# yuliangguo/OmniFusion

Measured on AMD Instinct MI355X. Metric: panoramas/sec at 512x1024 ERP, N=18 256^2 patches; equi2pers+pers2equi GB/s vs HBM peak, higher is better.
Workload: dtype f16x3 (fp16 hi/lo pairs, fp32 accumulate: fp32-class); 1 GPU; cfg2/cfg4 shard: 8 panoramas/GPU/step, 512x1024 ERP, fov 80, nrows 4 (18 patches); full single-pass spherical_fusion forward (confidence=True) at patch size 128 — the only size the reference network exists at (SURVEY 0.1); random-init weights (seed 42); inputs resident in HBM; resample pair at 18x256^2 reported in roofline_resample; per_gpu_batch=8, global_batch=8, parallelism=image-sharded x1, execution=3 forwards in flight per GPU on 3 streams (spherical_fusion.pipelined)

## Files before the change

include/omnifusion.h:

```cpp
#ifndef OMNIFUSION_H_
#define OMNIFUSION_H_

#include <stddef.h>
#include <stdint.h>

#ifdef __cplusplus
extern "C" {
#endif

#define OMNI_VERSION 200

enum omni_status {
    OMNI_OK = 0,
    OMNI_ERR_INVALID = 1,
    OMNI_ERR_HIP = 2,
    OMNI_ERR_UNSUPPORTED = 3
};

enum omni_layout { OMNI_LAYOUT_BCHWN = 0, OMNI_LAYOUT_BNCHW = 1, OMNI_LAYOUT_BNHWC = 2,
                   OMNI_LAYOUT_BCHNW = 3  };
enum omni_dtype { OMNI_F32 = 0, OMNI_F16 = 1 };

typedef void* omni_stream_t;
typedef struct omni_geometry omni_geometry_t;

int omni_version(void);
const char* omni_last_error(void);

int omni_set_option(const char* name, int value);
int omni_get_option(const char* name, int* value);

int omni_num_patches(int nrows);

int omni_patch_centers(int nrows, int which, float* center_p_host);

int omni_geometry_create(omni_geometry_t** out, int nrows, float fov_h, float fov_w,
                         int ph, int pw, int H, int W, omni_stream_t stream);
void omni_geometry_destroy(omni_geometry_t* g);
void omni_geometry_cache_clear(void);
int omni_geometry_cache_size(void);

int omni_equi2pers(const void* erp, void* pers, int dtype, int B, int C, int H, int W,
                   int ph, int pw, int nrows, float fov_h, float fov_w, int layout,
                   omni_stream_t stream);

int omni_equi2pers_aux(float* xyz, float* uv, int ph, int pw, int nrows, float fov_h, float fov_w,
                       omni_stream_t stream);

int omni_pers2equi(const void* pers, void* erp, int dtype, int B, int C, int ph, int pw,
                   int H, int W, int nrows, float fov_h, float fov_w, int layout,
                   omni_stream_t stream);

int omni_patches_to_planar(const void* src, void* dst, int dtype, int B, int C, int ph, int pw, int N, omni_stream_t stream);

int omni_pers2equi_conf(const void* pred_w, const void* conf, float* out, int dtype, int B,
                        int ph, int pw, int H, int W, int nrows, float fov_h, float fov_w,
                        int layout, omni_stream_t stream);

int omni_equi2pers_g(const omni_geometry_t* g, const void* erp, void* pers, int dtype, int B, int C,
                     int layout, omni_stream_t stream);
int omni_pers2equi_g(const omni_geometry_t* g, const void* pers, void* erp, int dtype, int B, int C,
                     int layout, omni_stream_t stream);

enum omni_act { OMNI_ACT_NONE = 0, OMNI_ACT_RELU = 1, OMNI_ACT_GELU = 2 };

int omni_equi2pers_bwd(const void* grad_pers, void* grad_erp, int dtype, int B, int C, int H, int W,
                       int ph, int pw, int nrows, float fov_h, float fov_w, int layout, omni_stream_t stream);
int omni_pers2equi_bwd(const void* grad_erp, void* grad_pers, int dtype, int B, int C, int ph, int pw,
                       int H, int W, int nrows, float fov_h, float fov_w, int layout, omni_stream_t stream);
int omni_conv2d_nhwc_f32(const float* src1, const float* src2, const float* wt, const float* bias,
                         const float* res, float* dst, int M, int H, int W, int C1, int C2, int Cout,
                         int KH, int KW, int stride, int pad, int act, omni_stream_t stream);
int omni_conv2d_splitk_plan(long long rows, int Cout, int ksteps);
int omni_conv2d_nhwc_f32_ws(const float* src1, const float* src2, const float* wt, const float* bias,
                            const float* res, float* dst, int M, int H, int W, int C1, int C2, int Cout,
                            int KH, int KW, int stride, int pad, int act, int splitk, float* ws, size_t ws_bytes,
                            omni_stream_t stream);
int omni_conv2d_nhwc_f16x3_ws(const float* src1, const float* src2, const void* wt16, const float* bias,
                              const float* res, float* dst, int M, int H, int W, int C1, int C2, int Cout,
                              int KH, int KW, int stride, int pad, int act, int splitk, float* ws, size_t ws_bytes,
                              omni_stream_t stream);
int omni_conv2d_sh_f16x3_ws(const void* src1, const void* src2, const void* wt16, const float* bias,
                            const void* res, void* dst, int fmt, int M, int H, int W, int C1, int C2, int Cout,
                            int KH, int KW, int stride, int pad, int act, int splitk, float* ws, size_t ws_bytes,
                            omni_stream_t stream);
int omni_gemm_rows_sh_f16x3(const void* x, const void* wt16r, const float* bias, const float* res, void* dst, int fmt,
                            int rows, int K, int N, int act, omni_stream_t stream);
int omni_gemm_rows_pack(const void* wt16, void* wt16r, int N, int K, omni_stream_t stream);
int omni_gemm_rows_ln_sh_f16x3(const float* x, const float* ln_weight, const float* ln_bias, float eps, const void* wt16r, const float* bias,
                               const float* res, void* dst, int fmt, int rows, int N, int act, omni_stream_t stream);
int omni_conv3x3_up2_sh_f16x3(const void* src, const void* wt16, const float* bias, void* dst, int fmt,
                              int M, int Hl, int Wl, int C, int Cout, int act, omni_stream_t stream);
size_t omni_up2_heads_scratch_bytes(int M, int P);
int omni_conv3x3_up2_heads_sh_f16x3(const void* src, const void* wt16, const float* bias, const void* heads_w16f, float bias_pred, float bias_weight,
                                    float* scratch, size_t scratch_bytes, float* out_a, float* out_c, int M, int P, int confidence, omni_stream_t stream);
int omni_conv3x3_up2_heads_sh_f16x1(const void* src, const void* wt16, const float* bias, const void* heads_w16f, float bias_pred, float bias_weight,
                                    float* scratch, size_t scratch_bytes, float* out_a, float* out_c, int M, int P, int confidence, omni_stream_t stream);
int omni_heads_pack_f16x3(const float* w_host, void* dst_host);
int omni_conv2d_sh_f16x3_post_ws(const void* src1, const void* src2, const void* wt16, const float* bias,
                                 const void* res, void* dst, int fmt, int M, int H, int W, int C1, int C2, int Cout,
                                 int KH, int KW, int stride, int pad, int act, int splitk, float* ws, size_t ws_bytes,
                                 const float* post, size_t post_elems, omni_stream_t stream);
int omni_wino_input_sh(const void* src, void* V, int M, int H, int W, int C, omni_stream_t stream);
int omni_conv3x3_wino_sh_f16x3(const void* V, const void* wt16, const float* bias, const void* res, void* dst, int fmt,
                               int M, int H, int W, int C, int Cout, int act, int splitk, float* ws, size_t ws_bytes, omni_stream_t stream);
int omni_sh_from_f32(const float* src, void* dst, size_t n, omni_stream_t stream);
int omni_sh_to_f32(const void* src, float* dst, size_t n, omni_stream_t stream);
int omni_sh_overflow(int* flag, int reset);
int omni_stem_f32(const float* src, const float* wt, const float* bias, float* dst, int M, int P, omni_stream_t stream);
int omni_maxpool3x3s2_f32(const float* src, float* dst, int M, int H, int W, int C, omni_stream_t stream);
int omni_upsample_bilinear_f32(const float* src, float* dst, int M, int H, int W, int C, int Ho, int Wo, omni_stream_t stream);
int omni_add_hw_f32(float* x, const float* y, int M, int HW, int C, omni_stream_t stream);
int omni_add_period_f32(float* x, const float* y, size_t total, size_t period, omni_stream_t stream);
int omni_stem_sh(const float* src, const float* wt, const float* bias, void* dst, int M, int P, omni_stream_t stream);
int omni_stem_sh_f16x3(const float* src, const void* wt16, const float* bias, void* dst, int M, int P, omni_stream_t stream);
int omni_stem_sh_f16x1(const float* src, const void* wt16, const float* bias, void* dst, int M, int P, omni_stream_t stream);
int omni_maxpool3x3s2_sh(const void* src, void* dst, int M, int H, int W, int C, omni_stream_t stream);
int omni_upsample_bilinear_sh(const void* src, void* dst, int M, int H, int W, int C, int Ho, int Wo, omni_stream_t stream);
int omni_up2_tapsum_sh(const float* y, const float* bias, void* dst, int M, int Hl, int Wl, int Cout, int act, omni_stream_t stream);
int omni_add_hw_sh(void* x, const float* y, int M, int HW, int C, omni_stream_t stream);
int omni_add_period_sh(void* x, const float* y, size_t total, size_t period, omni_stream_t stream);
int omni_layernorm512_sh(const float* x, const float* g, const float* b, void* y, int rows, float eps, omni_stream_t stream);
int omni_gemm_rows_slices_sh_f16x3(const void* x, const void* wt16r, float* parts, int rows, int K, int N, int slices, omni_stream_t stream);
int omni_gemm_rows_ln_parts_sh_f16x3(const float* parts, int nparts, const float* pbias, const float* pres, float* xout,
                                     const float* ln_weight, const float* ln_bias, float eps, const void* wt16r, const float* bias,
                                     void* dst, int fmt, int rows, int N, int act, omni_stream_t stream);
int omni_splitk_reduce_ln512(const float* parts, int nparts, const float* bias, const float* res, float* tok, const float* ln_weight, const float* ln_bias,
                             float eps, void* y, int fmt, int rows, omni_stream_t stream);
int omni_gemm_sh_f16x3_ln512_ws(const void* x, const void* wt16, const float* bias, const float* res, float* tok, const float* ln_g, const float* ln_b,
                                float eps, void* y, int fmt, int rows, int K, int splitk, float* ws, size_t ws_bytes, omni_stream_t stream);
int omni_attention_qkv_sh(const float* qkv, void* out, int B, int N, omni_stream_t stream);
int omni_token_pack_f32(const float* d, const float* pos, float* tok, int M, int N, int HW, int C, omni_stream_t stream);
int omni_layernorm512_f32(const float* x, const float* g, const float* b, float* y, int rows, float eps, omni_stream_t stream);
int omni_attention_f32(const float* q, const float* kv, float* out, int B, int N, omni_stream_t stream);
int omni_heads_f32(const float* x, const float* w, float bias_pred, float bias_weight, float* out_a, float* out_c,
                   int M, int P, int confidence, omni_stream_t stream);
int omni_mlp_points_f32(const float* xyz, const float* depth, const float* w1, const float* b1, const float* w2,
                        const float* b2, float* out, int Mo, int N, int HW, omni_stream_t stream);

int omni_masked_median_f32(const float* x, const float* mask, size_t n, unsigned* ws, float* out, omni_stream_t stream);
int omni_depth_metrics_f32(float* pred, const float* gt, const float* mask, const float* scale_num, const float* scale_den,
                           size_t n, double* ws, float* out, omni_stream_t stream);

size_t omni_semantic_workspace_bytes(size_t npix);
int omni_semantic_step_f32(const float* logits, const int64_t* target, int B, int C, size_t HW, int64_t ignore_index, int K,
                           void* workspace, float* loss, int64_t* pred, int64_t* confusion, omni_stream_t stream);
int omni_semantic_grad_f32(const float* logits, const int64_t* target, int B, int C, size_t HW, int64_t ignore_index,
                           const void* workspace, const float* grad_out, float* grad_logits, omni_stream_t stream);
int omni_confusion_matrix_i64(const int64_t* pred, const int64_t* gt, size_t n, int K, int64_t* confusion, int64_t* n_bad,
                              omni_stream_t stream);

int omni_preprocess_rgb_u8(const unsigned char* src_hwc, float* dst_chw, int B, int Hs, int Ws, int H, int W, omni_stream_t stream);
int omni_preprocess_depth_u16(const unsigned short* src, float* depth, unsigned char* mask, int B, int Hs, int Ws, int H, int W,
                              float min_depth, float max_depth, omni_stream_t stream);
int omni_png_info(const void* data, size_t nbytes, int* width, int* height, int* bit_depth, int* color_type);
int omni_png_decode(const void* data, size_t nbytes, void* dst, int H, int W, int kind);
int omni_png_decode_batch(const void* const* datas, const size_t* nbytes, void* const* dsts, int n, int H, int W, int kind, int threads);
int omni_zlib_inflate(const void* src, size_t nbytes, void* dst, size_t cap, size_t* produced, size_t* consumed);
int omni_png_checksums(const void* data, size_t nbytes, unsigned* crc32, unsigned* adler32);
size_t omni_berhu_workspace_bytes(int B);
int omni_berhu_loss_f32(const float* pred, const float* gt, const float* mask, const float* weights, int B, size_t per_item,
                        void* workspace, float* loss, omni_stream_t stream);
int omni_berhu_grad_f32(const float* pred, const float* gt, const float* mask, const float* weights, int B, size_t per_item,
                        const void* workspace, const float* grad_out, float* grad_pred, omni_stream_t stream);
int omni_pointcloud_ply_f32(const float* depth, const float* rgb, unsigned char* records, int B, int H, int W, omni_stream_t stream);

size_t omni_dibr_workspace_bytes(int B, int C, int H, int W);
int omni_splat_render_f32(const float* img, const float* depth, const float* coords, float max_depth,
                          float* recon, unsigned char* mask , int B, int C, int H, int W,
                          void* workspace, omni_stream_t stream);
int omni_dibr_f32(const float* img, const float* depth, const float* uvgrid, const float* sgrid, int grid_batched,
                  float baseline, int mode, float* recon, unsigned char* mask ,
                  int B, int C, int H, int W, void* workspace, omni_stream_t stream);
int omni_splat_render_wt_f32(const float* img, const float* depth, const float* coords, float max_depth,
                             float* recon, unsigned char* mask , float* wt, int B, int C, int H, int W,
                             void* workspace, omni_stream_t stream);
int omni_dibr_wt_f32(const float* img, const float* depth, const float* uvgrid, const float* sgrid, int grid_batched,
                     float baseline, int mode, float* recon, unsigned char* mask , float* wt,
                     int B, int C, int H, int W, void* workspace, omni_stream_t stream);
size_t omni_dibr_bwd_workspace_bytes(int B, int C, int H, int W);
int omni_splat_render_bwd_f32(const float* grad_recon, const float* recon, const float* wt, const float* img, const float* depth,
                              const float* coords, float max_depth, float* grad_img, float* grad_depth, float* grad_coords,
                              int B, int C, int H, int W, void* workspace, omni_stream_t stream);
int omni_dibr_bwd_f32(const float* grad_recon, const float* recon, const float* wt, const float* img, const float* depth,
                      const float* uvgrid, const float* sgrid, int grid_batched, float baseline, int mode,
                      float* grad_img, float* grad_depth, int B, int C, int H, int W, void* workspace, omni_stream_t stream);

int omni_ssim_f32(const float* pred, const float* gt, int B, int C, int H, int W, int window, const float* win, int mode,
                  float* ssim, omni_stream_t stream);
size_t omni_photometric_workspace_bytes(int B, int C, int H, int W);
size_t omni_photometric_grad_scratch_bytes(int B, int C, int H, int W);
int omni_photometric_loss_f32(const float* pred, const float* gt, const float* mask, int mask_c, const float* weights, int weights_c,
                              int B, int C, int H, int W, int window, const float* win, int mode, float alpha,
                              void* workspace, float* loss, omni_stream_t stream);
int omni_photometric_grad_f32(const float* pred, const float* gt, const float* mask, int mask_c, const float* weights, int weights_c,
                              int B, int C, int H, int W, int window, const float* win, int mode, float alpha,
                              const void* workspace, void* scratch, const float* grad_out, float* grad_pred, omni_stream_t stream);

int omni_freeview_rotations(const float* theta_deg, const float* phi_deg, int N, float* rot_fwd_host , float* rot_inv_host );
int omni_freeview_equi2pers_f32(const float* erp, float* pers, const float* rot_fwd_dev, int B, int C, int H, int W,
                                int N, int h, int w, float hfov_deg, float wfov_deg, int layout, omni_stream_t stream);
int omni_freeview_pers2equi_f32(const float* pers, float* erp, unsigned char* mask, const float* rot_inv_dev,
                                int N, int C, int h, int w, int H, int W, float hfov_deg, float wfov_deg, omni_stream_t stream);
int omni_freeview_merge_f32(const float* pers, float* erp, unsigned char* count, const float* rot_inv_dev,
                            int B, int N, int C, int h, int w, int H, int W, float hfov_deg, float wfov_deg, omni_stream_t stream);

size_t omni_freeview_bwd_workspace_bytes(int op, int items, int C, int Ht, int Wt);
int omni_freeview_equi2pers_bwd_f32(const float* grad_pers, float* grad_erp, const float* rot_fwd_dev, int B, int C, int H, int W,
                                    int N, int h, int w, float hfov_deg, float wfov_deg, int layout, void* ws, omni_stream_t stream);
int omni_freeview_pers2equi_bwd_f32(const float* grad_erp, float* grad_pers, const float* rot_inv_dev, int N, int C, int h, int w,
                                    int H, int W, float hfov_deg, float wfov_deg, void* ws, omni_stream_t stream);
int omni_freeview_merge_bwd_f32(const float* grad_erp, float* grad_pers, const float* rot_inv_dev, int B, int N, int C, int h, int w,
                                int H, int W, float hfov_deg, float wfov_deg, void* ws, omni_stream_t stream);

int omni_depth_normals_f32(const float* depth, const float* ray_tables, int B, int H, int W, float* normals, omni_stream_t stream);
int omni_sobel_f32(const float* img, int B, int C, int H, int W, float* grad_y, float* grad_x, omni_stream_t stream);
size_t omni_l1_workspace_bytes(int B);
int omni_l1_loss_f32(const float* pred, const float* gt, const float* mask, int B, int C, size_t hw, int mask_c, void* workspace,
                     float* loss, omni_stream_t stream);
int omni_l1_grad_f32(const float* pred, const float* gt, const float* mask, int B, int C, size_t hw, int mask_c, const void* workspace,
                     const float* grad_out, float* grad_pred, omni_stream_t stream);
size_t omni_geometry_terms_workspace_bytes(int B, int H, int W);
int omni_geometry_terms_f32(const float* pred, const float* gt, const float* mask, const float* ray_tables, int B, int H, int W, int terms,
                            int erode_mask, void* workspace, float* losses, omni_stream_t stream);
int omni_geometry_terms_grad_f32(const float* pred, const float* gt, const float* mask, const float* ray_tables, int B, int H, int W,
                                 int erode_mask, const void* workspace, const float* grad_normal, const float* grad_grad, float* grad_pred,
                                 omni_stream_t stream);

#ifdef __cplusplus
}
#endif
#endif
```

omnifusion_amd/_lib.py:

```python
import ctypes
import os

_HERE = os.path.dirname(os.path.abspath(__file__))
LIB_PATH = os.environ.get("OMNI_LIB_VARIANT") or os.path.join(_HERE, "csrc", "libomnifusion_hip.so")
LIB_PATH_DEBUG = os.path.join(_HERE, "csrc", "libomnifusion_hip_dbg.so")

OMNI_OK, OMNI_ERR_INVALID, OMNI_ERR_HIP, OMNI_ERR_UNSUPPORTED = 0, 1, 2, 3
LAYOUT_BCHWN, LAYOUT_BNCHW, LAYOUT_BNHWC, LAYOUT_BCHNW = 0, 1, 2, 3
F32, F16 = 0, 1

_lib = None


class OmniLibraryMissing(ImportError):
    pass


EXPORTS = [
    "omni_version", "omni_last_error", "omni_set_option", "omni_get_option", "omni_num_patches", "omni_patch_centers",
    "omni_geometry_create", "omni_geometry_destroy", "omni_geometry_cache_clear", "omni_geometry_cache_size",
    "omni_equi2pers", "omni_equi2pers_aux", "omni_pers2equi", "omni_pers2equi_conf", "omni_patches_to_planar",
    "omni_equi2pers_g", "omni_pers2equi_g", "omni_equi2pers_bwd", "omni_pers2equi_bwd",
    "omni_conv2d_nhwc_f32", "omni_stem_f32", "omni_maxpool3x3s2_f32", "omni_upsample_bilinear_f32",
    "omni_add_hw_f32", "omni_add_period_f32", "omni_token_pack_f32", "omni_layernorm512_f32",
    "omni_attention_f32", "omni_heads_f32", "omni_mlp_points_f32",
    "omni_conv2d_nhwc_f16x3_ws", "omni_conv2d_sh_f16x3_ws", "omni_conv2d_sh_f16x3_post_ws", "omni_gemm_rows_sh_f16x3", "omni_gemm_rows_ln_sh_f16x3", "omni_gemm_rows_pack", "omni_conv3x3_up2_sh_f16x3", "omni_conv3x3_up2_heads_sh_f16x3", "omni_conv3x3_up2_heads_sh_f16x1", "omni_up2_heads_scratch_bytes", "omni_heads_pack_f16x3", "omni_sh_from_f32", "omni_sh_to_f32", "omni_sh_overflow",
    "omni_stem_sh", "omni_stem_sh_f16x3", "omni_stem_sh_f16x1", "omni_maxpool3x3s2_sh", "omni_upsample_bilinear_sh", "omni_up2_tapsum_sh", "omni_add_hw_sh", "omni_add_period_sh", "omni_layernorm512_sh", "omni_gemm_sh_f16x3_ln512_ws", "omni_gemm_rows_slices_sh_f16x3", "omni_gemm_rows_ln_parts_sh_f16x3", "omni_splitk_reduce_ln512", "omni_wino_input_sh", "omni_conv3x3_wino_sh_f16x3", "omni_attention_qkv_sh",
    "omni_conv2d_splitk_plan", "omni_conv2d_nhwc_f32_ws",
    "omni_masked_median_f32", "omni_depth_metrics_f32",
    "omni_png_info", "omni_png_decode", "omni_png_decode_batch", "omni_zlib_inflate", "omni_png_checksums",
    "omni_preprocess_rgb_u8", "omni_preprocess_depth_u16", "omni_berhu_workspace_bytes", "omni_berhu_loss_f32", "omni_berhu_grad_f32",
    "omni_pointcloud_ply_f32",
    "omni_dibr_workspace_bytes", "omni_splat_render_f32", "omni_dibr_f32",
    "omni_splat_render_wt_f32", "omni_dibr_wt_f32", "omni_dibr_bwd_workspace_bytes", "omni_splat_render_bwd_f32", "omni_dibr_bwd_f32",
    "omni_ssim_f32", "omni_photometric_workspace_bytes", "omni_photometric_grad_scratch_bytes", "omni_photometric_loss_f32",
    "omni_photometric_grad_f32",
    "omni_freeview_rotations", "omni_freeview_equi2pers_f32", "omni_freeview_pers2equi_f32", "omni_freeview_merge_f32",
    "omni_freeview_bwd_workspace_bytes", "omni_freeview_equi2pers_bwd_f32", "omni_freeview_pers2equi_bwd_f32", "omni_freeview_merge_bwd_f32",
    "omni_semantic_workspace_bytes", "omni_semantic_step_f32", "omni_semantic_grad_f32", "omni_confusion_matrix_i64",
    "omni_depth_normals_f32", "omni_sobel_f32", "omni_l1_workspace_bytes", "omni_l1_loss_f32", "omni_l1_grad_f32",
    "omni_geometry_terms_workspace_bytes", "omni_geometry_terms_f32", "omni_geometry_terms_grad_f32",
]


def load():
    global _lib
    if _lib is not None:
        return _lib
    if not os.path.exists(LIB_PATH):
        raise OmniLibraryMissing(
            f"{LIB_PATH} not found: build it with `python -m omnifusion_amd.build` "
            "(hipcc --offload-arch=gfx950).  There is no fallback path.")
    import torch
    lib = ctypes.CDLL(LIB_PATH)
    lib.omni_last_error.restype = ctypes.c_char_p
    lib.omni_version.restype = ctypes.c_int
    lib.omni_up2_heads_scratch_bytes.restype = ctypes.c_size_t
    lib.omni_dibr_workspace_bytes.restype = ctypes.c_size_t
    lib.omni_splat_render_f32.argtypes = [ctypes.c_void_p] * 3 + [ctypes.c_float] + [ctypes.c_void_p] * 2 + [ctypes.c_int] * 4 + [ctypes.c_void_p] * 2
    lib.omni_dibr_f32.argtypes = [ctypes.c_void_p] * 4 + [ctypes.c_int, ctypes.c_float, ctypes.c_int] + [ctypes.c_void_p] * 2 + \
        [ctypes.c_int] * 4 + [ctypes.c_void_p] * 2
    vp, ci, cf = ctypes.c_void_p, ctypes.c_int, ctypes.c_float
    lib.omni_splat_render_wt_f32.argtypes = [vp] * 3 + [cf] + [vp] * 3 + [ci] * 4 + [vp] * 2
    lib.omni_dibr_wt_f32.argtypes = [vp] * 4 + [ci, cf, ci] + [vp] * 3 + [ci] * 4 + [vp] * 2
    lib.omni_dibr_bwd_workspace_bytes.restype = ctypes.c_size_t
    lib.omni_splat_render_bwd_f32.argtypes = [vp] * 6 + [cf] + [vp] * 3 + [ci] * 4 + [vp] * 2
    lib.omni_dibr_bwd_f32.argtypes = [vp] * 7 + [ci, cf, ci] + [vp] * 2 + [ci] * 4 + [vp] * 2
    lib.omni_ssim_f32.argtypes = [vp] * 2 + [ci] * 5 + [vp, ci, vp, vp]
    lib.omni_photometric_workspace_bytes.restype = ctypes.c_size_t
    lib.omni_photometric_grad_scratch_bytes.restype = ctypes.c_size_t
    lib.omni_photometric_loss_f32.argtypes = [vp, vp, vp, ci, vp, ci] + [ci] * 5 + [vp, ci, cf] + [vp] * 3
    lib.omni_photometric_grad_f32.argtypes = [vp, vp, vp, ci, vp, ci] + [ci] * 5 + [vp, ci, cf] + [vp] * 5
    lib.omni_freeview_rotations.argtypes = [vp, vp, ci, vp, vp]
    lib.omni_freeview_equi2pers_f32.argtypes = [vp] * 3 + [ci] * 7 + [cf, cf, ci, vp]
    lib.omni_freeview_pers2equi_f32.argtypes = [vp] * 4 + [ci] * 6 + [cf, cf, vp]
    lib.omni_freeview_merge_f32.argtypes = [vp] * 4 + [ci] * 7 + [cf, cf, vp]
    lib.omni_freeview_bwd_workspace_bytes.restype = ctypes.c_size_t
    lib.omni_freeview_bwd_workspace_bytes.argtypes = [ci] * 5
    lib.omni_freeview_equi2pers_bwd_f32.argtypes = [vp] * 3 + [ci] * 7 + [cf, cf, ci, vp, vp]
    lib.omni_freeview_pers2equi_bwd_f32.argtypes = [vp] * 3 + [ci] * 6 + [cf, cf, vp, vp]
    lib.omni_freeview_merge_bwd_f32.argtypes = [vp] * 3 + [ci] * 7 + [cf, cf, vp, vp]
    sz, i64 = ctypes.c_size_t, ctypes.c_int64
    lib.omni_semantic_workspace_bytes.restype = sz
    lib.omni_semantic_workspace_bytes.argtypes = [sz]
    lib.omni_semantic_step_f32.argtypes = [vp, vp, ci, ci, sz, i64, ci] + [vp] * 5
    lib.omni_semantic_grad_f32.argtypes = [vp, vp, ci, ci, sz, i64] + [vp] * 4
    lib.omni_confusion_matrix_i64.argtypes = [vp, vp, sz, ci] + [vp] * 3
    lib.omni_depth_normals_f32.argtypes = [vp, vp, ci, ci, ci, vp, vp]
    lib.omni_sobel_f32.argtypes = [vp] + [ci] * 4 + [vp] * 3
    lib.omni_l1_workspace_bytes.restype = sz
    lib.omni_l1_workspace_bytes.argtypes = [ci]
    lib.omni_l1_loss_f32.argtypes = [vp] * 3 + [ci, ci, sz, ci] + [vp] * 3
    lib.omni_l1_grad_f32.argtypes = [vp] * 3 + [ci, ci, sz, ci] + [vp] * 4
    lib.omni_geometry_terms_workspace_bytes.restype = sz
    lib.omni_geometry_terms_workspace_bytes.argtypes = [ci] * 3
    lib.omni_geometry_terms_f32.argtypes = [vp] * 4 + [ci] * 5 + [vp] * 3
    lib.omni_geometry_terms_grad_f32.argtypes = [vp] * 4 + [ci] * 4 + [vp] * 5
    for name in EXPORTS:
        getattr(lib, name)
    _lib = lib
    return lib


def load_debug():
    import torch
    if not os.path.exists(LIB_PATH_DEBUG):
        raise OmniLibraryMissing(f"{LIB_PATH_DEBUG} not found: python -m omnifusion_amd.build --debug")
    lib = ctypes.CDLL(LIB_PATH_DEBUG)
    lib.omni_last_error.restype = ctypes.c_char_p
    return lib


def set_option(name, value):
    check(load().omni_set_option(name.encode(), int(value)), "set_option")


def get_option(name):
    v = ctypes.c_int(0)
    check(load().omni_get_option(name.encode(), ctypes.byref(v)), "get_option")
    return v.value


CALL_LOG = None


def check(status, what=""):
    if CALL_LOG is not None:
        CALL_LOG.append(what)
    if status == OMNI_OK:
        return
    msg = load().omni_last_error().decode(errors="replace")
    if status == OMNI_ERR_INVALID:
        raise ValueError(f"{what}: {msg}")
    if status == OMNI_ERR_UNSUPPORTED:
        raise NotImplementedError(f"{what}: {msg}")
    raise RuntimeError(f"{what}: {msg}")


def ptr(t):
    return ctypes.c_void_p(t.data_ptr())


def stream_of(t):
    import torch
    return ctypes.c_void_p(torch.cuda.current_stream(t.device).cuda_stream)


def dtype_code(t):
    import torch
    if t.dtype == torch.float32:
        return F32
    if t.dtype == torch.float16:
        return F16
    raise ValueError(f"unsupported dtype {t.dtype}: the HIP path stores float32 or float16")
```

omnifusion_amd/csrc/omni_conv_sh.hip:

```cpp
#include "omni_conv_sh_common.h"

namespace {

__constant__ float wino_coef[16][4] = {
    {1, 0, 0, 0}, {1, 1, 0, 0}, {1, -1, 0, 0}, {0, -1, 0, 0},
    {1, 0, 1, 0}, {1, 1, 1, 1}, {1, -1, 1, -1}, {0, -1, 0, -1},
    {1, 0, -1, 0}, {1, 1, -1, -1}, {1, -1, -1, 1}, {0, -1, 0, 1},
    {0, 0, -1, 0}, {0, 0, -1, -1}, {0, 0, -1, 1}, {0, 0, 0, 1}};
template <int BM, int BN, int WM, int WN, int NST = 3, int NL = 0, bool PP = false, bool WINO = false, bool X1 = false>
__global__ __launch_bounds__(64 * (WM * WN + NL)) void conv_sh_kernel(ShConvArgs a)
{
    static_assert(!(WINO && X1), "Winograd: f16x3 only");
    static_assert(!PP || (NL > 0 && WM * WN == 8 && NST >= 3), "ping-pong: eight matrix waves (two per SIMD) + loader waves, three stages");
    static_assert(!WINO || (PP && BM / WM == 32 && BN / WN == 32), "Winograd: the ping-pong kernel with 32 x 32 wave tiles");
    constexpr int NW = WM * WN, LW = NL > 0 ? NL : NW, RPP = 8 * LW;
    constexpr int TM = BM / WM / 32, TN = BN / WN / 32;
    constexpr int APASS = BM / RPP, BPASS = BN / RPP, LPS = APASS + BPASS;
    static_assert(APASS >= 1 && BPASS >= 1, "a tile side must cover at least one DMA pass");
    constexpr int A_BYTES = BM * 128, STAGE = (BM + BN) * 128;
    __shared__ __attribute__((aligned(1024))) unsigned char lds[NST * STAGE];
    __shared__ long long cst[OMNI_ABL(32768) ? 256 : 1];
    const bool stamped = OMNI_ABL(32768) && blockIdx.x == 0 && blockIdx.y == 0 && a.ws != nullptr && a.splitk <= 1;
    auto cstamp = [&](int k) { if (OMNI_ABL(32768) && stamped && (threadIdx.x & 63) == 0 && k < 256) cst[k] = clock64(); };
    auto cdump = [&]() { if (OMNI_ABL(32768) && stamped && threadIdx.x == 0) for (int i = 0; i < 256; ++i) reinterpret_cast<long long*>(a.ws)[i] = cst[i]; };
    if (threadIdx.x == 0) cstamp(0);

    const int t = threadIdx.x, lane = t & 63;
    const int wave = __builtin_amdgcn_readfirstlane(t >> 6);
    const int wm = wave / WN, wn = wave % WN;
    const bool loader = NL > 0 && wave >= NW;
    const int iw = NL > 0 ? wave - NW : wave;
    const int ntn = a.Cout / BN;
    const int ntm = (a.rows + BM - 1) / BM;
    const unsigned lb = a.noxcd ? blockIdx.x : omni_xcd_remap(blockIdx.x, gridDim.x);
    const int tile_m = a.wt_major ? (int)(lb % (unsigned)ntm) : (int)(lb / (unsigned)ntn), tile_n = a.wt_major ? (int)(lb / (unsigned)ntm) : (int)(lb % (unsigned)ntn);
    const int row0 = tile_m * BM, col0 = tile_n * BN;
    const int G1 = a.C1 >> 5, G2 = a.C2 >> 5, G = G1 + G2;
    const int ksteps = a.KH * a.KW * G;

    const int gs = (lane & 15) ^ ((4 * iw + (lane >> 4)) & 15);
    const int rl = 8 * iw + 2 * (lane >> 4) + (gs >> 3), pc16 = (gs & 7) * 16;
    int pix[APASS];
    unsigned vmask[APASS];
#pragma unroll
    for (int i = 0; i < APASS; ++i) {
        const int r = row0 + rl + RPP * i;
        vmask[i] = 0; pix[i] = 0;
        if constexpr (WINO) {
            if ((NL == 0 || loader) && r < a.rows) { pix[i] = r; vmask[i] = 0xffffu; }
        } else
        if ((NL == 0 || loader) && r < a.rows) {
            const int hw = a.Ho * a.Wo;
            const int m = r / hw, rem = r - m * hw;
            const int oy = (rem / a.Wo) * a.stride - a.pad, ox = (rem % a.Wo) * a.stride - a.pad;
            pix[i] = (m * a.H + oy) * a.W + ox;
            unsigned vm = 0;
#pragma unroll
            for (int ky = 0; ky < 3; ++ky)
#pragma unroll
                for (int kx = 0; kx < 3; ++kx)
                    if (ky < a.KH && kx < a.KW && (unsigned)(oy + ky) < (unsigned)a.H && (unsigned)(ox + kx) < (unsigned)a.W)
                        vm |= 1u << (ky * a.KW + kx);
            vmask[i] = vm;
        }
    }
    const rsrc_t rs1 = make_rsrc(a.src1, (size_t)a.M * a.H * a.W * a.C1 * 4);
    const rsrc_t rs2 = make_rsrc(a.src2 ? a.src2 : a.src1, a.src2 ? (size_t)a.M * a.H * a.W * a.C2 * 4 : 0);
    const rsrc_t rsw = make_rsrc(a.wt, (size_t)a.Cout * ksteps * 128);
    int wbase[BPASS];
#pragma unroll
    for (int i = 0; i < BPASS; ++i) wbase[i] = (col0 + rl + RPP * i) * ksteps * 128 + pc16;

    int f_tap = 0, f_src = 0, f_gl = 0, f_ky = 0, f_kx = 0, f_gn = G1;
    int voff[APASS];
    auto refresh = [&]() {
        const int cs4 = (f_src ? a.C2 : a.C1) * 4;
        const int toff = (f_ky * a.W + f_kx) * cs4 + pc16;
#pragma unroll
        for (int i = 0; i < APASS; ++i)
            voff[i] = ((vmask[i] >> f_tap) & 1u) ? pix[i] * cs4 + toff : (int)0x80000000;
    };
    auto seek = [&](int ks) {
        f_tap = ks / G; const int g = ks - f_tap * G;
        f_src = g >= G1; f_gl = f_src ? g - G1 : g; f_gn = f_src ? G2 : G1;
        f_ky = f_tap / a.KW; f_kx = f_tap - f_ky * a.KW;
        refresh();
    };
    auto issue_a = [&](auto slot_c) {
        constexpr int SLOT = decltype(slot_c)::value;
        unsigned char* sb = lds + SLOT * STAGE + iw * 1024;
        const int so = f_gl * 128;
        if (OMNI_ABL(128)) {}
        else if (f_src) {
#pragma unroll
            for (int i = 0; i < APASS; ++i) dma16(rs2, sb + i * (1024 * LW), voff[i], so);
        } else {
#pragma unroll
            for (int i = 0; i < APASS; ++i) dma16(rs1, sb + i * (1024 * LW), voff[i], so);
        }
    };
    auto issue_b = [&](int ks, auto slot_c) {
        constexpr int SLOT = decltype(slot_c)::value;
        unsigned char* sb = lds + SLOT * STAGE + iw * 1024;
        if (!OMNI_ABL(128)) {
#pragma unroll
            for (int i = 0; i < BPASS; ++i) dma16(rsw, sb + A_BYTES + i * (1024 * LW), wbase[i], ks * 128);
        }
        if (++f_gl == f_gn) {
            f_gl = 0;
            if (f_src == 0 && G2 > 0) { f_src = 1; f_gn = G2; }
            else { f_src = 0; f_gn = G1; ++f_tap; if (++f_kx == a.KW) { f_kx = 0; ++f_ky; } }
            refresh();
        }
    };
    auto issue = [&](int ks, auto slot_c) { issue_a(slot_c); issue_b(ks, slot_c); };

    f16v acc[TM][TN], acc1[TM][TN];
#pragma unroll
    for (int i = 0; i < TM; ++i)
#pragma unroll
        for (int j = 0; j < TN; ++j) { acc[i][j] = (f16v)(0.0f); acc1[i][j] = (f16v)(0.0f); }

    int foa[4], fob[4];
    {
        const int r = lane & 31, v = r >> 1, h = lane >> 5;
#pragma unroll
        for (int k = 0; k < 4; ++k) {
            const int f = v * 256 + ((((r & 1) * 8 + 2 * k + h) ^ v) * 16);
            foa[k] = f + wm * (BM / WM) * 128;
            fob[k] = f + A_BYTES + wn * (BN / WN) * 128;
        }
    }

    int ks_begin = 0, ks_end = ksteps;
    if (a.splitk > 1) {
        const int per = (ksteps + a.splitk - 1) / a.splitk;
        ks_begin = (int)blockIdx.y * per; ks_end = min(ksteps, ks_begin + per);
    }
    if (NL == 0 || loader) {
        seek(ks_begin);
        [&]<int... S>(std::integer_sequence<int, S...>) {
            ((ks_begin + S < ks_end ? issue(ks_begin + S, std::integral_constant<int, S>()) : (void)0), ...);
        }(std::make_integer_sequence<int, NST - 1>());
    }
    auto pbarrier = [&]() {
        __builtin_amdgcn_sched_barrier(0);
        __builtin_amdgcn_s_barrier();
        asm volatile("" ::: "memory");
        __builtin_amdgcn_sched_barrier(0);
    };
    if (loader) {
        if constexpr (PP) {
            auto lstep = [&](int ks, auto slot_c) {
                constexpr int SLOT = decltype(slot_c)::value;
                const int sk_ = 128 + 4 * (ks - ks_begin);
                if (wave == NW && ks - ks_begin < 28) cstamp(sk_);
                if (ks + NST - 2 < ks_end) wait_vm<(NST - 2) * LPS>();
                else                       wait_vm<0>();
                if (wave == NW && ks - ks_begin < 28) cstamp(sk_ + 1);
                pbarrier();
                if (wave == NW && ks - ks_begin < 28) cstamp(sk_ + 2);
                if (ks + NST - 1 < ks_end) issue_a(std::integral_constant<int, (SLOT + NST - 1) % NST>());
                if (wave == NW && ks - ks_begin < 28) cstamp(sk_ + 3);
                pbarrier();
                if (ks + NST - 1 < ks_end) issue_b(ks + NST - 1, std::integral_constant<int, (SLOT + NST - 1) % NST>());
            };
            int ks = ks_begin;
            for (; ks + NST - 1 < ks_end; ks += NST) {
                [&]<int... S>(std::integer_sequence<int, S...>) { (lstep(ks + S, std::integral_constant<int, S>()), ...); }
                (std::make_integer_sequence<int, NST>());
            }
            [&]<int... S>(std::integer_sequence<int, S...>) {
                ((ks + S < ks_end ? lstep(ks + S, std::integral_constant<int, S>()) : (void)0), ...);
            }(std::make_integer_sequence<int, NST - 1>());
            pbarrier();
            if (!WINO && a.splitk <= 1 && a.dst_sh && !a.res_f32 && !a.post && a.epi_lds) __syncthreads();
            return;
        }
        auto lstep = [&](int ks, auto slot_c) {
            constexpr int SLOT = decltype(slot_c)::value;
            const int sk_ = 128 + 4 * (ks - ks_begin);
            if (wave == NW && ks - ks_begin < 28) cstamp(sk_);
            if (ks + NST - 2 < ks_end) wait_vm<(NST - 2) * LPS>();
            else                       wait_vm<0>();
            if (wave == NW && ks - ks_begin < 28) cstamp(sk_ + 1);
            __builtin_amdgcn_s_barrier();
            asm volatile("" ::: "memory");
            if (wave == NW && ks - ks_begin < 28) cstamp(sk_ + 2);
            if (ks + NST - 1 < ks_end) issue(ks + NST - 1, std::integral_constant<int, (SLOT + NST - 1) % NST>());
            if (wave == NW && ks - ks_begin < 28) cstamp(sk_ + 3);
        };
        int ks = ks_begin;
        for (; ks + NST - 1 < ks_end; ks += NST) {
            [&]<int... S>(std::integer_sequence<int, S...>) { (lstep(ks + S, std::integral_constant<int, S>()), ...); }
            (std::make_integer_sequence<int, NST>());
        }
        [&]<int... S>(std::integer_sequence<int, S...>) {
            ((ks + S < ks_end ? lstep(ks + S, std::integral_constant<int, S>()) : (void)0), ...);
        }(std::make_integer_sequence<int, NST - 1>());
        if (a.splitk <= 1 && a.dst_sh && !a.res_f32 && !a.post && a.epi_lds) __syncthreads();
        return;
    }

    if constexpr (PP) {
        const bool grp_b = wave >= NW / 2;
        h8v ah[2][TM], al[2][TM], bh[2][TN], bl[2][TN];
        auto reads = [&](auto slot_c) {
            constexpr int SLOT = decltype(slot_c)::value;
            const unsigned char* sl = lds + SLOT * STAGE;
#pragma unroll
            for (int kc = 0; kc < 2; ++kc) {
#pragma unroll
                for (int i = 0; i < TM; ++i) {
                    ah[kc][i] = *reinterpret_cast<const h8v*>(sl + i * 4096 + foa[kc]);
                    if constexpr (!X1) al[kc][i] = *reinterpret_cast<const h8v*>(sl + i * 4096 + foa[2 + kc]);
                }
#pragma unroll
                for (int j = 0; j < TN; ++j) {
                    bh[kc][j] = *reinterpret_cast<const h8v*>(sl + j * 4096 + fob[kc]);
                    if constexpr (!X1) bl[kc][j] = *reinterpret_cast<const h8v*>(sl + j * 4096 + fob[2 + kc]);
                }
            }
            wait_lds_reads();
        };
        auto mfmas = [&]() {
            if constexpr (OMNI_PP_PRIO) __builtin_amdgcn_s_setprio(1);
#pragma unroll
            for (int kc = 0; kc < 2; ++kc)
#pragma unroll
                for (int i = 0; i < TM; ++i)
#pragma unroll
                    for (int j = 0; j < TN; ++j) {
                        acc[i][j] = __builtin_amdgcn_mfma_f32_32x32x16_f16(bh[kc][j], ah[kc][i], acc[i][j], 0, 0, 0);
                        if constexpr (!X1) {
                            acc1[i][j] = __builtin_amdgcn_mfma_f32_32x32x16_f16(bl[kc][j], ah[kc][i], acc1[i][j], 0, 0, 0);
                            acc1[i][j] = __builtin_amdgcn_mfma_f32_32x32x16_f16(bh[kc][j], al[kc][i], acc1[i][j], 0, 0, 0);
                        }
                    }
            if constexpr (OMNI_PP_PRIO) __builtin_amdgcn_s_setprio(0);
        };
        f16v Y[WINO ? 4 : 1];
        int wino_g = 0, wino_p = ks_begin / (G > 0 ? G : 1);
        if constexpr (WINO) {
#pragma unroll
            for (int o = 0; o < 4; ++o) Y[o] = (f16v)(0.0f);
        }
        auto wino_fold = [&]() {
            if constexpr (WINO) {
                if (++wino_g < G) return;
                wino_g = 0;
                f16v m;
#pragma unroll
                for (int e = 0; e < 16; ++e) m[e] = fmaf(acc1[0][0][e], 4.8828125e-4f, acc[0][0][e]);
#pragma unroll
                for (int o = 0; o < 4; ++o) {
                    const float c = wino_coef[wino_p][o];
                    if (c != 0.0f) {
#pragma unroll
                        for (int e = 0; e < 16; ++e) Y[o][e] = fmaf(c, m[e], Y[o][e]);
                    }
                }
                acc[0][0] = (f16v)(0.0f); acc1[0][0] = (f16v)(0.0f);
                ++wino_p;
            }
        };
        pbarrier();
        if (!grp_b) {
            auto stepa = [&](int ks, auto slot_c) {
                if (wave == 0 && ks - ks_begin < 28) cstamp(8 + 4 * (ks - ks_begin));
                reads(slot_c);
                if (wave == 0 && ks - ks_begin < 28) cstamp(11 + 4 * (ks - ks_begin));
                pbarrier();
                if (wave == 0 && ks - ks_begin < 28) cstamp(9 + 4 * (ks - ks_begin));
                mfmas();
                wino_fold();
                if (wave == 0 && ks - ks_begin < 28) cstamp(10 + 4 * (ks - ks_begin));
                pbarrier();
            };
            int ks = ks_begin;
            for (; ks + NST - 1 < ks_end; ks += NST) {
                [&]<int... S>(std::integer_sequence<int, S...>) { (stepa(ks + S, std::integral_constant<int, S>()), ...); }
                (std::make_integer_sequence<int, NST>());
            }
            [&]<int... S>(std::integer_sequence<int, S...>) {
                ((ks + S < ks_end ? stepa(ks + S, std::integral_constant<int, S>()) : (void)0), ...);
            }(std::make_integer_sequence<int, NST - 1>());
        } else {
            auto stepb = [&](int ks, auto slot_c) {
                pbarrier();
                reads(slot_c);
                pbarrier();
                mfmas();
                wino_fold();
            };
            int ks = ks_begin;
            for (; ks + NST - 1 < ks_end; ks += NST) {
                [&]<int... S>(std::integer_sequence<int, S...>) { (stepb(ks + S, std::integral_constant<int, S>()), ...); }
                (std::make_integer_sequence<int, NST>());
            }
            [&]<int... S>(std::integer_sequence<int, S...>) {
                ((ks + S < ks_end ? stepb(ks + S, std::integral_constant<int, S>()) : (void)0), ...);
            }(std::make_integer_sequence<int, NST - 1>());
        }
        if constexpr (WINO) {
            const int tl = row0 + wm * (BM / WM) + (lane & 31);
            if (tl >= a.rows) return;
            const int per_img = a.wino_th * a.wino_tw, m = tl / per_img, rem = tl - m * per_img, ty = rem / a.wino_tw, tx = rem - ty * a.wino_tw;
            const int cj[1] = {col0 + wn * (BN / WN)};
#pragma unroll
            for (int o = 0; o < 4; ++o) {
                const size_t r = ((size_t)m * a.Ho + 2 * ty + (o >> 1)) * a.Wo + 2 * tx + (o & 1);
                if (a.splitk > 1) {
#pragma unroll
                    for (int q = 0; q < 4; ++q) {
                        f4v v; v.x = Y[o][4 * q]; v.y = Y[o][4 * q + 1]; v.z = Y[o][4 * q + 2]; v.w = Y[o][4 * q + 3];
                        *reinterpret_cast<f4v*>(a.ws + ((size_t)blockIdx.y * a.wino_pix + r) * a.Cout + cj[0] + 8 * q + 4 * (lane >> 5)) = v;
                    }
                } else {
                    const f16v ea[1] = {Y[o]}, eb[1] = {(f16v)(0.0f)};
                    epilogue_row<1, 2>(ea, eb, a, r, cj, lane, a.dst_sh != 0);
                }
            }
            return;
        }
    }
    auto step = [&](int ks, auto slot_c) {
        constexpr int SLOT = decltype(slot_c)::value;
        if (NL == 0) {
            if (ks + NST - 2 < ks_end) wait_vm<(NST - 2) * LPS>();
            else                       wait_vm<0>();
        }
        if (wave == 0 && ks - ks_begin < 28) cstamp(8 + 4 * (ks - ks_begin));
        wait_lds_reads();
        if (!OMNI_ABL(256)) __builtin_amdgcn_s_barrier();
        asm volatile("" ::: "memory");
        if (wave == 0 && ks - ks_begin < 28) cstamp(9 + 4 * (ks - ks_begin));
        const unsigned char* sl = lds + SLOT * STAGE;
        h8v ah[2][TM], al[2][TM], bh[2][TN], bl[2][TN];
        if (OMNI_ABL(512)) {
#pragma unroll
            for (int kc = 0; kc < 2; ++kc) {
#pragma unroll
                for (int i = 0; i < TM; ++i) { ah[kc][i] = (h8v)((_Float16)1.0f); al[kc][i] = ah[kc][i]; }
#pragma unroll
                for (int j = 0; j < TN; ++j) { bh[kc][j] = (h8v)((_Float16)1.0f); bl[kc][j] = bh[kc][j]; }
            }
        } else
#pragma unroll
        for (int kc = 0; kc < 2; ++kc) {
#pragma unroll
            for (int i = 0; i < TM; ++i) {
                ah[kc][i] = *reinterpret_cast<const h8v*>(sl + i * 4096 + foa[kc]);
                if constexpr (!X1) al[kc][i] = *reinterpret_cast<const h8v*>(sl + i * 4096 + foa[2 + kc]);
            }
#pragma unroll
            for (int j = 0; j < TN; ++j) {
                bh[kc][j] = *reinterpret_cast<const h8v*>(sl + j * 4096 + fob[kc]);
                if constexpr (!X1) bl[kc][j] = *reinterpret_cast<const h8v*>(sl + j * 4096 + fob[2 + kc]);
            }
        }
#pragma unroll
        for (int kc = 0; kc < 2; ++kc) {
            __builtin_amdgcn_sched_barrier(0);
#pragma unroll
            for (int i = 0; i < TM; ++i)
#pragma unroll
                for (int j = 0; j < TN; ++j) {
                    if (!OMNI_ABL(64) && !OMNI_DBG(a, 64)) acc[i][j] = __builtin_amdgcn_mfma_f32_32x32x16_f16(bh[kc][j], ah[kc][i], acc[i][j], 0, 0, 0);
                    else { acc[i][j][0] += (float)bh[kc][j][0] * (float)ah[kc][i][0]; }
                    if constexpr (!X1) {
                        if (!OMNI_ABL(16) && !OMNI_DBG(a, 16)) acc1[i][j] = __builtin_amdgcn_mfma_f32_32x32x16_f16(bl[kc][j], ah[kc][i], acc1[i][j], 0, 0, 0);
                        if (!OMNI_ABL(32) && !OMNI_DBG(a, 32)) acc1[i][j] = __builtin_amdgcn_mfma_f32_32x32x16_f16(bh[kc][j], al[kc][i], acc1[i][j], 0, 0, 0);
                    }
                }
            if (kc == 0) {
                __builtin_amdgcn_sched_barrier(0);
                if (NL == 0 && ks + NST - 1 < ks_end) issue(ks + NST - 1, std::integral_constant<int, (SLOT + NST - 1) % NST>());
            }
        }
    };
    if constexpr (!PP) {
        int ks = ks_begin;
        for (; ks + NST - 1 < ks_end; ks += NST) {
            [&]<int... S>(std::integer_sequence<int, S...>) { (step(ks + S, std::integral_constant<int, S>()), ...); }
            (std::make_integer_sequence<int, NST>());
        }
        [&]<int... S>(std::integer_sequence<int, S...>) {
            ((ks + S < ks_end ? step(ks + S, std::integral_constant<int, S>()) : (void)0), ...);
        }(std::make_integer_sequence<int, NST - 1>());
    }

    if (wave == 0) cstamp(1);
    if (OMNI_ABL(4) || OMNI_DBG(a, 4)) return;
    if (a.splitk <= 1 && a.dst_sh && !a.res_f32 && !a.post && a.epi_lds) {
        static_assert(NW * 32 * (32 * TN + 4) * 4 <= NST * STAGE, "the transposition tiles must fit the K loop's buffers");
        wait_lds_reads();
        __syncthreads();
        float* tile = reinterpret_cast<float*>(lds) + wave * (32 * (32 * TN + 4));
        int c0[TN];
#pragma unroll
        for (int j = 0; j < TN; ++j) c0[j] = col0 + wn * (BN / WN) + j * 32;
#pragma unroll
        for (int i = 0; i < TM; ++i) {
            const int r0 = row0 + wm * (BM / WM) + i * 32;
            if (r0 < a.rows) epilogue_tile_lds<TN, false, X1>(acc[i], acc1[i], a, (size_t)r0, min(32, a.rows - r0), c0, lane, tile);
            if (i + 1 < TM) asm volatile("s_waitcnt lgkmcnt(0)" ::: "memory");
        }
        if (OMNI_ABL(32768)) { if (wave == 0) cstamp(2); __syncthreads(); cdump(); }
        return;
    }
#pragma unroll
    for (int i = 0; i < TM; ++i) {
        const int r = row0 + wm * (BM / WM) + i * 32 + (lane & 31);
        if (r >= a.rows) continue;
        if (a.splitk > 1) {
#pragma unroll
            for (int j = 0; j < TN; ++j)
#pragma unroll
                for (int q = 0; q < 4; ++q) {
                    const int c = col0 + wn * (BN / WN) + j * 32 + 8 * q + 4 * (lane >> 5);
                    f4v v;
#pragma unroll
                    for (int e = 0; e < 4; ++e) v[e] = acc_join<X1>(acc1[i][j][4 * q + e], acc[i][j][4 * q + e]);
                    *reinterpret_cast<f4v*>(a.ws + ((size_t)blockIdx.y * a.rows + r) * a.Cout + c) = v;
                }
        } else {
            if constexpr (NL > 0 && TN > 1) {
#pragma unroll
                for (int j = 0; j < TN; ++j) {
                    const f16v ea[1] = {acc[i][j]}, eb[1] = {acc1[i][j]};
                    const int cj[1] = {col0 + wn * (BN / WN) + j * 32};
                    epilogue_row<1, 2, X1>(ea, eb, a, (size_t)r, cj, lane, a.dst_sh != 0);
                }
            } else {
                int c0[TN];
#pragma unroll
                for (int j = 0; j < TN; ++j) c0[j] = col0 + wn * (BN / WN) + j * 32;
                epilogue_row<TN, 4, X1>(acc[i], acc1[i], a, (size_t)r, c0, lane, a.dst_sh != 0);
            }
        }
    }
}

__global__ __launch_bounds__(256) void sh_splitk_reduce_kernel(const float* __restrict__ ws, const float* __restrict__ bias,
                                                               const void* __restrict__ res, void* __restrict__ dst,
                                                               size_t n4, int Cout, int splitk, size_t slab, int act, int dst_sh, int res_f32)
{
    const size_t i = (size_t)blockIdx.x * 256 + threadIdx.x;
    if (i >= n4) return;
    const size_t o = i * 4;
    f4v v = *reinterpret_cast<const f4v*>(ws + o);
    for (int s = 1; s < splitk; ++s) v += *reinterpret_cast<const f4v*>(ws + (size_t)s * slab + o);
    splitk_finish(v, o, bias, res, dst, Cout, act, dst_sh, res_f32);
}

template <bool SH>
__global__ __launch_bounds__(256) void sh_splitk_reduce_ln512_kernel(const float* __restrict__ ws, const float* __restrict__ bias, const float* __restrict__ res,
                                                                     float* __restrict__ tok, const float* __restrict__ g, const float* __restrict__ b,
                                                                     void* __restrict__ y, int rows, int splitk, size_t slab, float eps)
{
    const int row = blockIdx.x * 4 + (threadIdx.x >> 6), lane = threadIdx.x & 63;
    if (row >= rows) return;
    const size_t o = (size_t)row * 512;
    f4v v0 = *reinterpret_cast<const f4v*>(ws + o + lane * 4), v1 = *reinterpret_cast<const f4v*>(ws + o + 256 + lane * 4);
    for (int s = 1; s < splitk; ++s) {
        v0 += *reinterpret_cast<const f4v*>(ws + (size_t)s * slab + o + lane * 4);
        v1 += *reinterpret_cast<const f4v*>(ws + (size_t)s * slab + o + 256 + lane * 4);
    }
    if (bias) { v0 += *reinterpret_cast<const f4v*>(bias + lane * 4); v1 += *reinterpret_cast<const f4v*>(bias + 256 + lane * 4); }
    if (res) { v0 += *reinterpret_cast<const f4v*>(res + o + lane * 4); v1 += *reinterpret_cast<const f4v*>(res + o + 256 + lane * 4); }
    *reinterpret_cast<f4v*>(tok + o + lane * 4) = v0; *reinterpret_cast<f4v*>(tok + o + 256 + lane * 4) = v1;
    float sum = (v0.x + v0.y) + (v0.z + v0.w) + (v1.x + v1.y) + (v1.z + v1.w);
#pragma unroll
    for (int d = 32; d > 0; d >>= 1) sum += __shfl_xor(sum, d);
    const float mean = sum * (1.0f / 512.0f);
    v0 -= mean; v1 -= mean;
    float q = (v0.x * v0.x + v0.y * v0.y) + (v0.z * v0.z + v0.w * v0.w) + (v1.x * v1.x + v1.y * v1.y) + (v1.z * v1.z + v1.w * v1.w);
#pragma unroll
    for (int d = 32; d > 0; d >>= 1) q += __shfl_xor(q, d);
    const float rstd = 1.0f / sqrtf(q * (1.0f / 512.0f) + eps);
    const f4v g0 = *reinterpret_cast<const f4v*>(g + lane * 4), g1 = *reinterpret_cast<const f4v*>(g + 256 + lane * 4);
    const f4v b0 = *reinterpret_cast<const f4v*>(b + lane * 4), b1 = *reinterpret_cast<const f4v*>(b + 256 + lane * 4);
    act_store4<SH>(y, o + lane * 4, v0 * rstd * g0 + b0);
    act_store4<SH>(y, o + 256 + lane * 4, v1 * rstd * g1 + b1);
}

__global__ __launch_bounds__(256) void sh_from_f32_kernel(const float* __restrict__ src, void* __restrict__ dst, size_t n4)
{
    const size_t i = (size_t)blockIdx.x * 256 + threadIdx.x;
    if (i >= n4) return;
    h4v hi, lo; sh_split4(*reinterpret_cast<const f4v*>(src + i * 4), hi, lo);
    unsigned char* dp = (unsigned char*)dst + sh_off(i * 4);
    *reinterpret_cast<h4v*>(dp) = hi; *reinterpret_cast<h4v*>(dp + 64) = lo;
}
__global__ __launch_bounds__(256) void sh_to_f32_kernel(const void* __restrict__ src, float* __restrict__ dst, size_t n4)
{
    const size_t i = (size_t)blockIdx.x * 256 + threadIdx.x;
    if (i >= n4) return;
    const unsigned char* sp = (const unsigned char*)src + sh_off(i * 4);
    *reinterpret_cast<f4v*>(dst + i * 4) = sh_join4(*reinterpret_cast<const h4v*>(sp), *reinterpret_cast<const h4v*>(sp + 64));
}

template <bool X1, int BM, int BN, int WM, int WN, int NST = 3, int NL = 0>
void launch_sh(ShConvArgs a, hipStream_t s)
{
    const int tiles = ((a.rows + BM - 1) / BM) * (a.Cout / BN);
    if constexpr (NL > 0 && WM * WN == 8) {
        if (omni_options().conv_pingpong) {
            hipLaunchKernelGGL((conv_sh_kernel<BM, BN, WM, WN, NST, NL, true, false, X1>), dim3(tiles, a.splitk > 1 ? a.splitk : 1), dim3(64 * (WM * WN + NL)), 0, s, a);
            return;
        }
    }
    hipLaunchKernelGGL((conv_sh_kernel<BM, BN, WM, WN, NST, NL, false, false, X1>), dim3(tiles, a.splitk > 1 ? a.splitk : 1), dim3(64 * (WM * WN + NL)), 0, s, a);
}

}

static int conv2d_sh_impl(const void* src1, const void* src2, const void* wt16, const float* bias,
                          const void* res, void* dst, int fmt, int M, int H, int W, int C1, int C2, int Cout,
                          int KH, int KW, int stride, int pad, int act, int splitk, float* ws, size_t ws_bytes,
                          const float* post, size_t post_elems, omni_stream_t stream, bool reduce = true);
extern "C" int omni_conv2d_sh_f16x3_ws(const void* src1, const void* src2, const void* wt16, const float* bias,
                                       const void* res, void* dst, int fmt, int M, int H, int W, int C1, int C2, int Cout,
                                       int KH, int KW, int stride, int pad, int act, int splitk, float* ws, size_t ws_bytes,
                                       omni_stream_t stream)
{
    return conv2d_sh_impl(src1, src2, wt16, bias, res, dst, fmt, M, H, W, C1, C2, Cout, KH, KW, stride, pad, act, splitk, ws, ws_bytes,
                          nullptr, 0, stream);
}
extern "C" int omni_conv2d_sh_f16x3_post_ws(const void* src1, const void* src2, const void* wt16, const float* bias,
                                            const void* res, void* dst, int fmt, int M, int H, int W, int C1, int C2, int Cout,
                                            int KH, int KW, int stride, int pad, int act, int splitk, float* ws, size_t ws_bytes,
                                            const float* post, size_t post_elems, omni_stream_t stream)
{
    return conv2d_sh_impl(src1, src2, wt16, bias, res, dst, fmt, M, H, W, C1, C2, Cout, KH, KW, stride, pad, act, splitk, ws, ws_bytes,
                          post, post_elems, stream);
}
extern "C" int omni_gemm_sh_f16x3_ln512_ws(const void* x, const void* wt16, const float* bias, const float* res, float* tok, const float* ln_g, const float* ln_b,
                                           float eps, void* y, int fmt, int rows, int K, int splitk, float* ws, size_t ws_bytes, omni_stream_t stream)
{
    if (!x || !wt16 || !tok || !ln_g || !ln_b || !y) OMNI_FAIL(OMNI_ERR_INVALID, "omni_gemm_sh_f16x3_ln512: null pointer");
    if (rows <= 0 || K <= 0 || K % 32) OMNI_FAIL(OMNI_ERR_INVALID, "omni_gemm_sh_f16x3_ln512: bad shape");
    if (fmt & 8) OMNI_FAIL(OMNI_ERR_UNSUPPORTED, "omni_gemm_sh_f16x3_ln512: no f16x1 form (fmt bit 3)");
    const int S = std::min(splitk, K / 32);
    if (S < 2) OMNI_FAIL(OMNI_ERR_INVALID, "omni_gemm_sh_f16x3_ln512: needs a split-K plan (splitk >= 2); an unsplit GEMM writes its result in its own epilogue");
    const int rc = conv2d_sh_impl(x, nullptr, wt16, bias, res, tok, 2, rows, 1, 1, K, 0, 512, 1, 1, 1, 0, OMNI_ACT_NONE, S, ws, ws_bytes, nullptr, 0, stream, false);
    if (rc != OMNI_OK) return rc;
    hipStream_t s = (hipStream_t)stream;
    if (fmt & 1) hipLaunchKernelGGL(sh_splitk_reduce_ln512_kernel<true>, dim3((rows + 3) / 4), dim3(256), 0, s, (const float*)ws, bias, res, tok, ln_g, ln_b, y, rows, S, (size_t)rows * 512, eps);
    else         hipLaunchKernelGGL(sh_splitk_reduce_ln512_kernel<false>, dim3((rows + 3) / 4), dim3(256), 0, s, (const float*)ws, bias, res, tok, ln_g, ln_b, y, rows, S, (size_t)rows * 512, eps);
    OMNI_HIP(hipGetLastError());
    return OMNI_OK;
}

template <bool X1>
static void conv_sh_select(const ShConvArgs& a, int fmt, hipStream_t s)
{
    const int KH = a.KH, KW = a.KW, stride = a.stride, pad = a.pad, H = a.H, W = a.W, M = a.M, Cout = a.Cout;
    const int ksteps = KH * KW * ((a.C1 + a.C2) / 32);
    const long long rows = a.rows;
    if (a.splitk <= 1 && KH == 3 && KW == 3 && stride == 1 && pad == 1 && H == W && (W == 16 || (W == 8 && omni_options().conv_img >= 2)) && rows % 128 == 0 &&
        Cout % 64 == 0 && !(fmt & 4) && omni_options().conv_img > 0 && !omni_options().conv_nohalo) {
        const int grid = (int)(rows / 128) * (Cout / 64);
        if (omni_options().conv_halo_bn == 32) {
            if (W == 16) omni_halo_launch(&a, 32, 4, false, 16, X1, 2 * grid, s);
            else         omni_halo_launch(&a, 32, 4, false, 8, X1, 2 * grid, s);
        }
        else if (W == 16) omni_halo_launch(&a, 64, 4, false, 16, X1, grid, s);
        else         omni_halo_launch(&a, 64, 4, false, 8, X1, grid, s);
        return;
    }
    if (a.splitk <= 1 && KH == 3 && KW == 3 && stride == 1 && pad == 1 && W % HT_W == 0 && H % 4 == 0 && !omni_options().conv_nohalo) {
        const int th = (H % 8 == 0 && omni_options().conv_halo_th == 8) ? 8 : 4;
        const int grid = M * (H / th) * (W / HT_W);
        if (th == 8) {
            if (Cout % 64 == 0 && omni_options().conv_halo_bn != 32) omni_halo_launch(&a, 64, 8, false, 0, X1, grid * (Cout / 64), s);
            else                omni_halo_launch(&a, 32, 8, false, 0, X1, grid * (Cout / 32), s);
        } else {
            const bool bn32 = omni_options().conv_halo_bn == 32 || ((fmt & 4) && omni_options().conv_halo_bn_lat == 32);
            if (Cout % 64 == 0 && !bn32) omni_halo_launch(&a, 64, 4, false, 0, X1, grid * (Cout / 64), s);
            else                omni_halo_launch(&a, 32, 4, false, 0, X1, grid * (Cout / 32), s);
        }
        return;
    }
    int tile = omni_options().conv_sh_tile;
    if (tile < 0) tile = 8;
    if (Cout % 64 != 0) launch_sh<X1, 128, 32, 4, 1>(a, s);
    else if (tile == 2 && Cout % 128 == 0) launch_sh<X1, 128, 128, 2, 2>(a, s);
    else if (tile == 1) launch_sh<X1, 128, 64, 2, 2>(a, s);
    else if (tile == 3) launch_sh<X1, 128, 64, 4, 2>(a, s);
    else if (tile == 4 && Cout % 128 == 0) launch_sh<X1, 128, 128, 4, 2>(a, s);
    else if (tile == 8 && Cout % 128 == 0 && ((rows + 255) / 256) * (long long)(Cout / 128) * a.splitk >= std::max(1, omni_options().conv_big_blocks)) launch_sh<X1, 256, 128, 4, 2>(a, s);
    else if (tile == 8 && Cout % 128 == 0 && ((rows + 127) / 128) * (long long)(Cout / 128) * a.splitk >= 128) launch_sh<X1, 128, 128, 4, 2, 3, 4>(a, s);
    else if (tile == 8 && ((rows + 127) / 128) * (long long)(Cout / 64) * a.splitk >= 128) launch_sh<X1, 128, 64, 4, 2, 3, 4>(a, s);
    else if (tile == 9 && Cout % 128 == 0 && ((rows + 255) / 256) * (long long)(Cout / 128) * a.splitk >= 128) launch_sh<X1, 256, 128, 4, 2>(a, s);
    else if (tile == 9 && Cout % 128 == 0 && ((rows + 127) / 128) * (long long)(Cout / 128) * a.splitk >= 128) launch_sh<X1, 128, 128, 4, 2>(a, s);
    else if (tile == 9 && ((rows + 127) / 128) * (long long)(Cout / 64) * a.splitk >= 128) launch_sh<X1, 128, 64, 4, 2>(a, s);
    else if (tile >= 5 && tile <= 7 && Cout % 128 == 0 && ((rows + 127) / 128) * (long long)(Cout / 128) * a.splitk >= (32ll << (tile - 4))) launch_sh<X1, 128, 128, 4, 2>(a, s);
    else if (tile >= 5 && tile <= 7 && ((rows + 127) / 128) * (long long)(Cout / 64) * a.splitk >= (32ll << (tile - 4))) launch_sh<X1, 128, 64, 4, 2>(a, s);
    else if (((rows + 63) / 64) * (long long)(Cout / 64) * a.splitk <= 256 && ksteps >= 8 && !omni_options().conv_nodeep) {
        if (omni_options().conv_deep_loaders) launch_sh<X1, 64, 64, 2, 2, 6, 4>(a, s);
        else launch_sh<X1, 64, 64, 2, 2, 6>(a, s);
    }
    else launch_sh<X1, 64, 64, 2, 2>(a, s);
}

static int conv2d_sh_impl(const void* src1, const void* src2, const void* wt16, const float* bias,
                          const void* res, void* dst, int fmt, int M, int H, int W, int C1, int C2, int Cout,
                          int KH, int KW, int stride, int pad, int act, int splitk, float* ws, size_t ws_bytes,
                          const float* post, size_t post_elems, omni_stream_t stream, bool reduce)
{
    const int dst_sh = fmt & 1;
    if (!src1 || !wt16 || !dst) OMNI_FAIL(OMNI_ERR_INVALID, "omni_conv2d_sh: null pointer");
    if (C1 <= 0 || C1 % 32 || C2 < 0 || C2 % 32 || Cout <= 0 || Cout % 32 || (C2 > 0 && !src2))
        OMNI_FAIL(OMNI_ERR_INVALID, "omni_conv2d_sh: channels must be multiples of 32");
    if (M <= 0 || H <= 0 || W <= 0 || KH <= 0 || KW <= 0 || KH > 3 || KW > 3 || stride <= 0 || pad < 0)
        OMNI_FAIL(OMNI_ERR_INVALID, "omni_conv2d_sh: bad shape (kernels up to 3x3)");
    ShConvArgs a;
    a.src1 = src1; a.src2 = src2; a.wt = wt16; a.bias = bias; a.res = res; a.dst = dst; a.dst_sh = dst_sh; a.res_f32 = (fmt >> 1) & 1;
    a.dbg = 0; a.noxcd = omni_options().conv_noxcd; a.wt_major = 0; a.epi_lds = omni_options().conv_epi_lds && !(fmt & 4);
#ifdef OMNI_DEBUG_BUILD
    a.dbg = omni_debug_bits("OMNI_CONV_DBG");
#endif
    a.M = M; a.H = H; a.W = W; a.C1 = C1; a.C2 = C2; a.Cout = Cout;
    a.KH = KH; a.KW = KW; a.stride = stride; a.pad = pad; a.act = act;
    a.Ho = (H + 2 * pad - KH) / stride + 1; a.Wo = (W + 2 * pad - KW) / stride + 1;
    const long long rows = (long long)M * a.Ho * a.Wo;
    if (rows <= 0 || rows >= (1ll << 31) || (long long)M * H * W >= (1ll << 31))
        OMNI_FAIL(OMNI_ERR_UNSUPPORTED, "omni_conv2d_sh: too many pixels for 32-bit row indices");
    a.rows = (int)rows;
    const int ksteps = KH * KW * ((C1 + C2) / 32);
    if ((long long)M * H * W * (C1 > C2 ? C1 : C2) * 4 >= (1ll << 31) || (long long)Cout * ksteps * 128 >= (1ll << 31))
        OMNI_FAIL(OMNI_ERR_UNSUPPORTED, "omni_conv2d_sh: an operand of 2 GiB or more (32-bit buffer offsets)");
    int S = splitk;
    if (S > ksteps) S = ksteps;
    if (S > 1 && (!ws || ws_bytes < (size_t)S * rows * Cout * sizeof(float)))
        OMNI_FAIL(OMNI_ERR_INVALID, "omni_conv2d_sh: split-K workspace too small");
    a.splitk = S > 1 ? S : 1; a.ws = ws;
    a.wt_major = omni_options().conv_wt_major == 2 || (omni_options().conv_wt_major == 1 &&
                 (long long)Cout * ksteps * 128 > (long long)M * H * W * (C1 + C2) * 4) ? 1 : 0;
    a.post = post; a.post_rows = 1; a.wino_th = a.wino_tw = a.wino_pix = 0;
    if (post) {
        if (Cout <= 0 || post_elems == 0 || post_elems % (size_t)Cout || post_elems / (size_t)Cout > 0x7fffffffull)
            OMNI_FAIL(OMNI_ERR_INVALID, "omni_conv2d_sh: the post-activation addend must hold whole rows of Cout channels");
        if (a.splitk > 1) OMNI_FAIL(OMNI_ERR_UNSUPPORTED, "omni_conv2d_sh: no post-activation addend with split-K");
        a.post_rows = (unsigned)(post_elems / (size_t)Cout);
    }
    hipStream_t s = (hipStream_t)stream;
    if (fmt & 8) conv_sh_select<true>(a, fmt, s);
    else         conv_sh_select<false>(a, fmt, s);
    OMNI_HIP(hipGetLastError());
    if (a.splitk > 1 && reduce) {
        const size_t n4 = (size_t)rows * Cout / 4;
        hipLaunchKernelGGL(sh_splitk_reduce_kernel, dim3((unsigned)((n4 + 255) / 256)), dim3(256), 0, s, (const float*)ws, bias, res, dst,
                           n4, Cout, a.splitk, (size_t)rows * Cout, act, a.dst_sh, a.res_f32);
        OMNI_HIP(hipGetLastError());
    }
    return OMNI_OK;
}

extern "C" int omni_splitk_reduce_ln512(const float* parts, int nparts, const float* bias, const float* res, float* tok, const float* lg, const float* lb,
                                        float eps, void* y, int fmt, int rows, omni_stream_t stream)
{
    if (!parts || nparts < 1 || !tok || !lg || !lb || !y || rows <= 0) OMNI_FAIL(OMNI_ERR_INVALID, "omni_splitk_reduce_ln512: null pointer or empty input");
    hipStream_t s = (hipStream_t)stream;
    if (fmt & 1) hipLaunchKernelGGL(sh_splitk_reduce_ln512_kernel<true>, dim3((rows + 3) / 4), dim3(256), 0, s, parts, bias, res, tok, lg, lb, y, rows, nparts, (size_t)rows * 512, eps);
    else         hipLaunchKernelGGL(sh_splitk_reduce_ln512_kernel<false>, dim3((rows + 3) / 4), dim3(256), 0, s, parts, bias, res, tok, lg, lb, y, rows, nparts, (size_t)rows * 512, eps);
    OMNI_HIP(hipGetLastError());
    return OMNI_OK;
}

OMNI_SH_OVERFLOW_ACCESSOR(omni_sh_overflow_conv)

extern "C" int omni_sh_overflow(int* flag, int reset)
{
    if (!flag) OMNI_FAIL(OMNI_ERR_INVALID, "omni_sh_overflow: null output");
    OMNI_HIP(hipDeviceSynchronize());
    unsigned v = 0;
    if (omni_sh_overflow_conv(&v, reset) != 0 || omni_sh_overflow_halo(&v, reset) != 0 || omni_sh_overflow_up2(&v, reset) != 0 ||
        omni_sh_overflow_rows(&v, reset) != 0 || omni_sh_overflow_net(&v, reset) != 0)
        OMNI_FAIL(OMNI_ERR_HIP, "omni_sh_overflow: could not read the device flag");
    *flag = v ? 1 : 0;
    return OMNI_OK;
}

extern "C" int omni_sh_from_f32(const float* src, void* dst, size_t n, omni_stream_t stream)
{
    if (!src || !dst || n % 32) OMNI_FAIL(OMNI_ERR_INVALID, "omni_sh_from_f32: null pointer or n % 32 != 0");
    if (n == 0) return OMNI_OK;
    hipLaunchKernelGGL(sh_from_f32_kernel, dim3((unsigned)((n / 4 + 255) / 256)), dim3(256), 0, (hipStream_t)stream, src, dst, n / 4);
    OMNI_HIP(hipGetLastError());
    return OMNI_OK;
}
extern "C" int omni_sh_to_f32(const void* src, float* dst, size_t n, omni_stream_t stream)
{
    if (!src || !dst || n % 32) OMNI_FAIL(OMNI_ERR_INVALID, "omni_sh_to_f32: null pointer or n % 32 != 0");
    if (n == 0) return OMNI_OK;
    hipLaunchKernelGGL(sh_to_f32_kernel, dim3((unsigned)((n / 4 + 255) / 256)), dim3(256), 0, (hipStream_t)stream, src, dst, n / 4);
    OMNI_HIP(hipGetLastError());
    return OMNI_OK;
}

namespace {

__global__ __launch_bounds__(256) void wino_input_sh_kernel(const void* __restrict__ src, void* __restrict__ V, int M, int H, int W, int C, size_t nt)
{
    const size_t i = (size_t)blockIdx.x * 256 + threadIdx.x;
    const int cq = C >> 2;
    if (i >= nt * cq) return;
    const size_t tl = i / cq;
    const int c = (int)(i - tl * cq) * 4;
    const int tw = W >> 1, th = H >> 1;
    const int m = (int)(tl / (size_t)(th * tw)), rem = (int)(tl - (size_t)m * th * tw), ty = rem / tw, tx = rem - ty * tw;
    f4v d[4][4];
#pragma unroll
    for (int a_ = 0; a_ < 4; ++a_)
#pragma unroll
        for (int b_ = 0; b_ < 4; ++b_) {
            const int y = 2 * ty - 1 + a_, x = 2 * tx - 1 + b_;
            d[a_][b_] = ((unsigned)y < (unsigned)H && (unsigned)x < (unsigned)W) ? act_load4<true>(src, (((size_t)m * H + y) * W + x) * C + c) : (f4v)(0.0f);
        }
    f4v u[4][4];
#pragma unroll
    for (int b_ = 0; b_ < 4; ++b_) { u[0][b_] = d[0][b_] - d[2][b_]; u[1][b_] = d[1][b_] + d[2][b_]; u[2][b_] = d[2][b_] - d[1][b_]; u[3][b_] = d[1][b_] - d[3][b_]; }
#pragma unroll
    for (int xi = 0; xi < 4; ++xi) {
        const f4v v0 = u[xi][0] - u[xi][2], v1 = u[xi][1] + u[xi][2], v2 = u[xi][2] - u[xi][1], v3 = u[xi][1] - u[xi][3];
        act_store4<true>(V, ((size_t)(4 * xi + 0) * nt + tl) * C + c, v0);
        act_store4<true>(V, ((size_t)(4 * xi + 1) * nt + tl) * C + c, v1);
        act_store4<true>(V, ((size_t)(4 * xi + 2) * nt + tl) * C + c, v2);
        act_store4<true>(V, ((size_t)(4 * xi + 3) * nt + tl) * C + c, v3);
    }
}

}

extern "C" int omni_wino_input_sh(const void* src, void* V, int M, int H, int W, int C, omni_stream_t stream)
{
    if (!src || !V) OMNI_FAIL(OMNI_ERR_INVALID, "omni_wino_input_sh: null pointer");
    if (M <= 0 || H <= 0 || W <= 0 || (H & 1) || (W & 1) || C <= 0 || C % 32) OMNI_FAIL(OMNI_ERR_INVALID, "omni_wino_input_sh: even image sides, channels a multiple of 32");
    const size_t nt = (size_t)M * (H / 2) * (W / 2), n = nt * (C / 4);
    if (16 * nt * C * 4 >= (1ull << 31)) OMNI_FAIL(OMNI_ERR_UNSUPPORTED, "omni_wino_input_sh: the transformed tensor must stay under 2 GiB (32-bit buffer offsets)");
    hipLaunchKernelGGL(wino_input_sh_kernel, dim3((unsigned)((n + 255) / 256)), dim3(256), 0, (hipStream_t)stream, src, V, M, H, W, C, nt);
    OMNI_HIP(hipGetLastError());
    return OMNI_OK;
}

extern "C" int omni_conv3x3_wino_sh_f16x3(const void* V, const void* wt16, const float* bias, const void* res, void* dst, int fmt,
                                          int M, int H, int W, int C, int Cout, int act, int splitk, float* ws, size_t ws_bytes, omni_stream_t stream)
{
    if (!V || !wt16 || !dst) OMNI_FAIL(OMNI_ERR_INVALID, "omni_conv3x3_wino_sh: null pointer");
    if (M <= 0 || H <= 0 || W <= 0 || (H & 1) || (W & 1) || C <= 0 || C % 32 || Cout <= 0 || Cout % 64) OMNI_FAIL(OMNI_ERR_INVALID, "omni_conv3x3_wino_sh: even image sides, C % 32 == 0, Cout % 64 == 0");
    if (splitk != 1 && splitk != 2 && splitk != 4) OMNI_FAIL(OMNI_ERR_INVALID, "omni_conv3x3_wino_sh: splitk must be 1, 2 or 4 (it divides the sixteen positions)");
    if (fmt & 8) OMNI_FAIL(OMNI_ERR_UNSUPPORTED, "omni_conv3x3_wino_sh: no f16x1 form (fmt bit 3)");
    const long long nt = (long long)M * (H / 2) * (W / 2), pix = (long long)M * H * W;
    if (16 * nt * C * 4 >= (1ll << 31) || (long long)Cout * 16 * C * 4 >= (1ll << 31) || pix >= (1ll << 31)) OMNI_FAIL(OMNI_ERR_UNSUPPORTED, "omni_conv3x3_wino_sh: an operand of 2 GiB or more");
    if (splitk > 1 && (!ws || ws_bytes < (size_t)splitk * pix * Cout * sizeof(float))) OMNI_FAIL(OMNI_ERR_INVALID, "omni_conv3x3_wino_sh: split workspace too small");
    ShConvArgs a;
    a.src1 = V; a.src2 = nullptr; a.wt = wt16; a.bias = bias; a.res = res; a.dst = dst; a.dst_sh = fmt & 1; a.res_f32 = (fmt >> 1) & 1;
    a.dbg = 0; a.noxcd = omni_options().conv_noxcd; a.wt_major = 0; a.epi_lds = 0;
    a.M = 1; a.H = 16; a.W = (int)nt; a.C1 = C; a.C2 = 0; a.Cout = Cout; a.KH = 16; a.KW = 1; a.stride = 1; a.pad = 0; a.act = act;
    a.Ho = H; a.Wo = W; a.rows = (int)nt; a.splitk = splitk; a.ws = ws; a.post = nullptr; a.post_rows = 1;
    a.wino_th = H / 2; a.wino_tw = W / 2; a.wino_pix = (int)pix;
    hipStream_t s = (hipStream_t)stream;
    const int tiles = (int)((nt + 127) / 128) * (Cout / 64);
    hipLaunchKernelGGL((conv_sh_kernel<128, 64, 4, 2, 3, 4, true, true>), dim3(tiles, splitk), dim3(64 * 12), 0, s, a);
    OMNI_HIP(hipGetLastError());
    if (splitk > 1) {
        const size_t n4 = (size_t)pix * Cout / 4;
        hipLaunchKernelGGL(sh_splitk_reduce_kernel, dim3((unsigned)((n4 + 255) / 256)), dim3(256), 0, s, (const float*)ws, bias, res, dst,
                           n4, Cout, splitk, (size_t)pix * Cout, act, a.dst_sh, a.res_f32);
        OMNI_HIP(hipGetLastError());
    }
    return OMNI_OK;
}
```

omnifusion_amd/model/_engine.py:

```python
import ctypes
import os

import torch

from .. import _lib
from ..equi_pers.equi2pers_v3 import equi2pers_patches, equi2pers_aux, pair, _NPATCH
from ..equi_pers.pers2equi_v3 import pers2equi, pers2equi_conf

ACT_NONE, ACT_RELU, ACT_GELU = 0, 1, 2
_LAYERS = [("layer1", 3, 1), ("layer2", 4, 2), ("layer3", 6, 2), ("layer4", 3, 2)]
_BN_EPS = 1e-5
PRECISIONS = ("f16x3", "f16x1", "fp32")


def _p(t):
    return ctypes.c_void_p(t.data_ptr()) if t is not None else None


def split_weights_f16x3(w):
    w = w.to(torch.float32)
    wmax = float(w.abs().max()) if w.numel() else 0.0
    if not wmax < 65504.0:
        raise ValueError(f"folded weight magnitude {wmax:g} is outside the fp16 range of the f16x3 operand format: "
                         "run this checkpoint with OMNI_NET_PRECISION=fp32")
    hi = w.half()
    hi = torch.where(w.abs() < 6.103515625e-05, torch.zeros_like(hi), hi)
    lo = ((w - hi.float()) * 2048.0).half()
    co, k = w.shape
    return torch.stack([hi.reshape(co, k // 32, 32), lo.reshape(co, k // 32, 32)], 2).contiguous()


def strip_module_prefix(sd):
    return {(k[7:] if k.startswith("module.") else k): v for k, v in sd.items()}


class Engine:
    def __init__(self, nrows, npatches, patch_size, fov, iterative, precision=None):
        self.nrows, self.npatches, self.iterative = nrows, npatches, iterative
        self.patch_size = pair(patch_size)
        self.fov = pair(fov)
        if self.patch_size[0] != self.patch_size[1]:
            raise ValueError("square patches only")
        self.w = None
        self.device = None
        self.precision = precision if precision is not None else os.environ.get("OMNI_NET_PRECISION", "f16x3")

    @property
    def sh(self):
        return self.precision in ("f16x3", "f16x1")

    @property
    def terms(self):
        return {"f16x3": 3, "f16x1": 1}.get(self.precision, 0)

    @property
    def _x1(self):
        return 8 if self.terms == 1 else 0

    def lane(self):
        e = Engine(self.nrows, self.npatches, self.patch_size, self.fov, self.iterative, precision=self.precision)
        e.w, e.device, e.head_bias = self.w, self.device, getattr(self, "head_bias", None)
        return e

    @staticmethod
    def _fold(sd, conv, bn):
        w = sd[conv + ".weight"].double()
        if w.dim() == 5:
            w = w[..., 0]
        g = sd[bn + ".weight"].double() / torch.sqrt(sd[bn + ".running_var"].double() + _BN_EPS)
        b = sd[bn + ".bias"].double() - sd[bn + ".running_mean"].double() * g
        return w * g[:, None, None, None], b

    @staticmethod
    def _gemm_layout(w):
        return w.permute(0, 2, 3, 1).reshape(w.shape[0], -1)

    def pack(self, state_dict, device):
        sd = {k: v.detach().cpu() for k, v in strip_module_prefix(state_dict).items()}
        dev = torch.device(device)
        f = lambda t: t.to(torch.float32).contiguous().to(dev)
        W = {}
        w, b = self._fold(sd, "conv1", "bn1")
        W["stem.w"] = f(w.permute(2, 3, 1, 0).reshape(147, 64)); W["stem.b"] = f(b)
        wk = torch.zeros((64, 3, 7, 8), dtype=torch.float64); wk[..., :7] = w
        W["stem.w16"] = split_weights_f16x3(torch.cat([wk.reshape(64, 168), torch.zeros((64, 24), dtype=torch.float64)], 1)).to(dev)

        def convbn(key, conv, bn):
            w, b = self._fold(sd, conv, bn)
            wg = self._gemm_layout(w).to(torch.float32)
            W[key + ".w"] = f(wg); W[key + ".b"] = f(b)
            W[key + ".w16"] = split_weights_f16x3(wg).to(dev)
        for lname, nblk, _ in _LAYERS:
            for i in range(nblk):
                p = f"{lname}.{i}"
                convbn(p + ".c1", p + ".conv1", p + ".bn1")
                convbn(p + ".c2", p + ".conv2", p + ".bn2")
                if (p + ".downsample.0.weight") in sd:
                    convbn(p + ".ds", p + ".downsample.0", p + ".downsample.1")
        for name in ("de_conv0_0", "de_conv0_1", "de_conv1_0", "de_conv1_1", "de_conv2_0", "de_conv2_1",
                     "de_conv3_0", "de_conv3_1", "de_conv4_0"):
            convbn(name, name + ".conv", name + ".bn")
        for name in ("de_conv0_0", "de_conv1_0"):
            w, _ = self._fold(sd, name + ".conv", name + ".bn")
            W[name + ".taps.w16"] = split_weights_f16x3(w.permute(2, 3, 0, 1).reshape(9 * w.shape[0], w.shape[1]).to(torch.float32)).to(dev)
        down = "down1" if self.iterative else "down"
        W["down.w"] = f(sd[down + ".weight"].reshape(32, 512)); W["down.b"] = f(sd[down + ".bias"])
        W["down.w16"] = split_weights_f16x3(sd[down + ".weight"].reshape(32, 512)).to(dev)
        W["pos"] = f(sd["transformer.pos_emb"].reshape(self.npatches, 512))
        for i in range(6):
            p = f"transformer.layer.{i}"
            for k in ("norm1.weight", "norm1.bias", "norm2.weight", "norm2.bias", "attn.q.weight", "attn.kv.weight",
                      "attn.proj.weight", "attn.proj.bias", "mlp.fc1.weight", "mlp.fc1.bias", "mlp.fc2.weight", "mlp.fc2.bias"):
                W[f"t{i}.{k}"] = f(sd[f"{p}.{k}"])
        for i in range(6):
            t = f"t{i}."
            W[t + "attn.qkv.w16"] = split_weights_f16x3(torch.cat([W[t + "attn.q.weight"], W[t + "attn.kv.weight"]], 0).cpu()).to(dev)
            for k in ("attn.proj", "mlp.fc1", "mlp.fc2"):
                W[t + k + ".w16"] = split_weights_f16x3(W[t + k + ".weight"].cpu()).to(dev)
        W["enc_norm.w"] = f(sd["transformer.encoder_norm.weight"]); W["enc_norm.b"] = f(sd["transformer.encoder_norm.bias"])
        hw = torch.stack([sd["pred.weight"][0, :, :, :, 0], sd["weight_pred.weight"][0, :, :, :, 0]])
        W["heads.w"] = f(hw.permute(0, 2, 3, 1).reshape(2, 9, 32))
        import numpy as np
        hw_host = np.ascontiguousarray(hw.permute(0, 2, 3, 1).reshape(2, 9, 32).to(torch.float32).numpy())
        frag = np.zeros(4 * 64 * 8, np.float16)
        _lib.check(_lib.load().omni_heads_pack_f16x3(hw_host.ctypes.data_as(ctypes.c_void_p), frag.ctypes.data_as(ctypes.c_void_p)), "heads_pack")
        W["heads.w16f"] = torch.from_numpy(frag).to(dev)
        self.head_bias = (float(sd["pred.bias"][0]), float(sd["weight_pred.bias"][0]))

        def mlp(name):
            w1, b1 = self._fold(sd, name + ".0", name + ".1")
            w2, b2 = self._fold(sd, name + ".3", name + ".4")
            return w1[:, :, 0, 0], b1, w2[:, :, 0, 0], b2
        P4 = self.patch_size[0] // 4
        if self.iterative:
            for name in ("mlp_points1", "mlp_points2"):
                w1, b1, w2, b2 = mlp(name)
                W[name + ".w1"], W[name + ".b1"], W[name + ".w2"], W[name + ".b2"] = f(w1), f(b1), f(w2), f(b2)
        else:
            cp = (ctypes.c_float * (2 * self.npatches))()
            _lib.check(_lib.load().omni_patch_centers(int(self.nrows), 0, cp), "patch_centers")
            c = torch.tensor(list(cp), dtype=torch.float64).reshape(self.npatches, 2)
            x = torch.cat([c, torch.ones(self.npatches, 1, dtype=torch.float64), c], 1)
            w1, b1, w2, b2 = mlp("mlp_points")
            h = torch.relu(x @ w1.T + b1)
            pf = torch.relu(h @ w2.T + b2)
            W["point_feat"] = f(pf[:, None, None, :].expand(self.npatches, P4, P4, 64))
        self.w, self.device = W, dev

    def read_overflow_flag(self, reset=True):
        if self.device is None:
            return False
        flag = ctypes.c_int(0)
        with torch.cuda.device(self.device):
            _lib.check(_lib.load().omni_sh_overflow(ctypes.byref(flag), 1 if reset else 0), "sh_overflow")
        return bool(flag.value)

    def _conv(self, x, key, M, H, Wd, C1, Cout, k, stride, pad, act, x2=None, C2=0, res=None, bias=True, out_f32=False, out=None, post=None):
        lib = _lib.load()
        Ho = (H + 2 * pad - k) // stride + 1
        Wo = (Wd + 2 * pad - k) // stride + 1
        if out is None:
            out = torch.empty((M, Ho, Wo, Cout), dtype=torch.float32, device=x.device)
        S, ws, nb = self._splitk(M * Ho * Wo, Cout, k * k * (C1 + C2) // 32, x.device, shape=(k, k, stride, pad, H, Wd))
        b = _p(self.w[key + ".b"]) if bias else None
        late_post = None
        if post is not None and (S > 1 or not self.sh or out_f32):
            late_post, post = post, None
        if self.sh and post is not None:
            rc = lib.omni_conv2d_sh_f16x3_post_ws(_p(x), _p(x2), _p(self.w[key + ".w16"]), b, _p(res), _p(out), (0 if out_f32 else 1) | self._x1,
                                                  M, H, Wd, C1, C2, Cout, k, k, stride, pad, act, S, _p(ws), ctypes.c_size_t(nb),
                                                  _p(post), ctypes.c_size_t(post.numel()), self._s)
        elif self.sh:
            lat = 4 if (self._bs == 1 and self.latency_plan) else 0
            rc = lib.omni_conv2d_sh_f16x3_ws(_p(x), _p(x2), _p(self.w[key + ".w16"]), b, _p(res), _p(out), (0 if out_f32 else 1) | lat | self._x1,
                                             M, H, Wd, C1, C2, Cout, k, k, stride, pad, act, S, _p(ws), ctypes.c_size_t(nb), self._s)
        else:
            rc = lib.omni_conv2d_nhwc_f32_ws(_p(x), _p(x2), _p(self.w[key + ".w"]), b, _p(res), _p(out), M, H, Wd, C1, C2, Cout,
                                             k, k, stride, pad, act, S, _p(ws), ctypes.c_size_t(nb), self._s)
        _lib.check(rc, "conv2d " + key)
        if late_post is not None:
            _lib.check((lib.omni_add_period_f32 if (out_f32 or not self.sh) else lib.omni_add_period_sh)(
                _p(out), _p(late_post), ctypes.c_size_t(out.numel()), ctypes.c_size_t(late_post.numel()), self._s), "add post " + key)
        return out

    NOMINAL_BATCH = 8
    SINGLE_BATCH = 4
    latency_plan = True
    rows_gemm = True

    def _splitk(self, rows, Cout, ksteps, device, shape=None):
        plan_batch = self.SINGLE_BATCH if (self._bs == 1 and self.latency_plan) else self.NOMINAL_BATCH
        rows_plan = rows // self._bs * plan_batch
        lib = _lib.load()
        S = int(lib.omni_conv2d_splitk_plan(ctypes.c_longlong(rows_plan), Cout, ksteps))
        if S <= 1:
            return 1, None, 0
        ws, nb = self._workspace(S * rows * Cout * 4, device)
        return S, ws, nb

    def _workspace(self, nbytes, device):
        nbytes = int(nbytes)
        if nbytes == 0:
            return None, 0
        ws = getattr(self, "_ws", None)
        if ws is None or ws.numel() * 4 < nbytes or ws.device != device:
            if ws is not None:
                self._ws_retired = getattr(self, "_ws_retired", []) + [ws]
            self._ws = ws = torch.empty((nbytes + 3) // 4, dtype=torch.float32, device=device)
        return ws, ws.numel() * 4

    def _gemm(self, x, wkey, bkey, rows, K, Nout, act=ACT_NONE, res=None):
        lib = _lib.load()
        out = torch.empty((rows, Nout), dtype=torch.float32, device=x.device)
        S, ws, nb = self._splitk(rows, Nout, K // 32, x.device)
        rc = lib.omni_conv2d_nhwc_f32_ws(_p(x), None, _p(self.w[wkey]), _p(self.w[bkey]) if bkey else None, _p(res), _p(out),
                                         rows, 1, 1, K, 0, Nout, 1, 1, 1, 0, act, S, _p(ws), ctypes.c_size_t(nb), self._s)
        _lib.check(rc, "gemm " + wkey)
        return out

    def _rows_weights(self, w16key, Nout, K):
        key = w16key + ".rows"
        w = self.w.get(key)
        if w is None:
            src = self.w[w16key]
            w = torch.empty_like(src)
            _lib.check(_lib.load().omni_gemm_rows_pack(_p(src), _p(w), Nout, K, self._s), "gemm_rows_pack")
            if not torch.cuda.is_current_stream_capturing():
                torch.cuda.current_stream(src.device).synchronize()
            self.w[key] = w
        return w

    def _gemm_sh(self, x, w16key, bkey, rows, K, Nout, act=ACT_NONE, res=None, out_sh=False):
        lib = _lib.load()
        out = torch.empty((rows, Nout), dtype=torch.float32, device=x.device)
        if self._bs == 1 and self.latency_plan and self.rows_gemm and rows <= 32 and K in (512, 2048):
            _lib.check(lib.omni_gemm_rows_sh_f16x3(_p(x), _p(self._rows_weights(w16key, Nout, K)), _p(self.w[bkey]) if bkey else None, _p(res), _p(out),
                                                   1 if out_sh else 0, rows, K, Nout, act, self._s), "gemm " + w16key)
            return out
        S, ws, nb = (1, None, 0) if K <= 512 else self._splitk(rows, Nout, K // 32, x.device)
        rc = lib.omni_conv2d_sh_f16x3_ws(_p(x), None, _p(self.w[w16key]), _p(self.w[bkey]) if bkey else None, _p(res), _p(out),
                                         (1 if out_sh else 0) | 2, rows, 1, 1, K, 0, Nout, 1, 1, 1, 0, act, S, _p(ws),
                                         ctypes.c_size_t(nb), self._s)
        _lib.check(rc, "gemm " + w16key)
        return out

    fuse_fc2_ln = os.environ.get("OMNI_FUSE_FC2_LN", "1") != "0"

    fc2_slices = int(os.environ.get("OMNI_FC2_SLICES", "4"))

    def _fc2_ln(self, h, w16key, bkey, rows, tok, nxt):
        lone = self._bs == 1 and self.latency_plan and self.rows_gemm and rows <= 32
        if lone and self.fc2_slices > 1 and self.fuse_ln:
            S = self.fc2_slices
            parts = torch.empty((S, rows, 512), dtype=torch.float32, device=h.device)
            _lib.check(_lib.load().omni_gemm_rows_slices_sh_f16x3(_p(h), _p(self._rows_weights(w16key, 512, 2048)), _p(parts), rows, 2048, 512, S, self._s), "gemm slices " + w16key)
            return None, None, (parts, S, bkey, tok)
        S, ws, nb = (1, None, 0) if lone else self._splitk(rows, 512, 2048 // 32, h.device)
        if lone or S <= 1 or not self.fuse_fc2_ln:
            return self._gemm_sh(h, w16key, bkey, rows, 2048, 512, res=tok), None, None
        wk, bk, eps, out_sh = nxt
        out, y = torch.empty((rows, 512), dtype=torch.float32, device=h.device), torch.empty((rows, 512), dtype=torch.float32, device=h.device)
        rc = _lib.load().omni_gemm_sh_f16x3_ln512_ws(_p(h), _p(self.w[w16key]), _p(self.w[bkey]), _p(tok), _p(out), _p(self.w[wk]), _p(self.w[bk]), ctypes.c_float(eps),
                                                     _p(y), 1 if out_sh else 0, rows, 2048, S, _p(ws), ctypes.c_size_t(nb), self._s)
        _lib.check(rc, "gemm+ln " + w16key)
        return out, y, None

    def _ln_gemm_parts(self, pending, lnw, lnb, eps, w16key, rows, Nout):
        parts, S, bkey, res_tok = pending
        tok = torch.empty((rows, 512), dtype=torch.float32, device=parts.device)
        out = torch.empty((rows, Nout), dtype=torch.float32, device=parts.device)
        rc = _lib.load().omni_gemm_rows_ln_parts_sh_f16x3(_p(parts), S, _p(self.w[bkey]), _p(res_tok), _p(tok), _p(self.w[lnw]), _p(self.w[lnb]), ctypes.c_float(eps),
                                                          _p(self._rows_weights(w16key, Nout, 512)), None, _p(out), 0, rows, Nout, ACT_NONE, self._s)
        _lib.check(rc, "ln+gemm (slices) " + w16key)
        return tok, out

    fuse_ln = os.environ.get("OMNI_FUSE_LN", "1") != "0"

    def _ln_gemm_sh(self, x, lnw, lnb, eps, w16key, bkey, rows, Nout, act=ACT_NONE, out_sh=False):
        if self._bs == 1 and self.latency_plan and self.rows_gemm and self.fuse_ln and rows <= 32:
            lib = _lib.load()
            out = torch.empty((rows, Nout), dtype=torch.float32, device=x.device)
            _lib.check(lib.omni_gemm_rows_ln_sh_f16x3(_p(x), _p(self.w[lnw]), _p(self.w[lnb]), ctypes.c_float(eps), _p(self._rows_weights(w16key, Nout, 512)),
                                                      _p(self.w[bkey]) if bkey else None, None, _p(out), 1 if out_sh else 0, rows, Nout, act, self._s), "ln+gemm " + w16key)
            return out
        return self._gemm_sh(self._ln_sh(x, lnw, lnb, rows, eps), w16key, bkey, rows, 512, Nout, act=act, out_sh=out_sh)

    def _ln_sh(self, x, wk, bk, rows, eps):
        y = torch.empty_like(x)
        _lib.check(_lib.load().omni_layernorm512_sh(_p(x), _p(self.w[wk]), _p(self.w[bk]), _p(y), rows, ctypes.c_float(eps), self._s), "layernorm")
        return y

    def _ln(self, x, wk, bk, rows, eps):
        y = torch.empty_like(x)
        _lib.check(_lib.load().omni_layernorm512_f32(_p(x), _p(self.w[wk]), _p(self.w[bk]), _p(y), rows, ctypes.c_float(eps), self._s), "layernorm")
        return y

    def _up(self, x, M, H, Wd, C, Ho, Wo):
        y = torch.empty((M, Ho, Wo, C), dtype=torch.float32, device=x.device)
        fn = _lib.load().omni_upsample_bilinear_sh if self.sh else _lib.load().omni_upsample_bilinear_f32
        _lib.check(fn(_p(x), _p(y), M, H, Wd, C, Ho, Wo, self._s), "upsample")
        return y

    fold_point_feat = True
    fuse_up = True

    def _up_conv(self, x, key, M, H, Wd, C, Cout, act, out_f32=False, out=None):
        Ho, Wo = 2 * H, 2 * Wd
        if self.sh and self.fuse_up and Wo % 32 == 0 and Ho % 4 == 0:
            if out is None:
                out = torch.empty((M, Ho, Wo, Cout), dtype=torch.float32, device=x.device)
            _lib.check(_lib.load().omni_conv3x3_up2_sh_f16x3(_p(x), _p(self.w[key + ".w16"]), _p(self.w[key + ".b"]), _p(out),
                                                             (0 if out_f32 else 1) | (4 if (self._bs == 1 and self.latency_plan) else 0) | self._x1,
                                                             M, H, Wd, C, Cout, act, self._s), "up+conv " + key)
            return out
        return self._conv(self._up(x, M, H, Wd, C, Ho, Wo), key, M, Ho, Wo, C, Cout, 3, 1, 1, act, out_f32=out_f32, out=out)

    taps_first = frozenset(("de_conv0_0",))

    def _up_conv_taps(self, x, key, M, H, Wd, C, Cout, act):
        if key in self.taps_first and self.sh and self.terms == 3 and Cout % 32 == 0 and H * Wd <= 64:
            y = self._conv(x, key + ".taps", M, H, Wd, C, 9 * Cout, 1, 1, 0, ACT_NONE, bias=False, out_f32=True)
            out = torch.empty((M, 2 * H, 2 * Wd, Cout), dtype=torch.float32, device=x.device)
            _lib.check(_lib.load().omni_up2_tapsum_sh(_p(y), _p(self.w[key + ".b"]), _p(out), M, H, Wd, Cout, act, self._s), "tap sum " + key)
            return out
        return self._conv(self._up(x, M, H, Wd, C, 2 * H, 2 * Wd), key, M, 2 * H, 2 * Wd, C, Cout, 3, 1, 1, act)

    def transformer(self, d, bs):
        lib = _lib.load()
        dev = d.device
        self._s = ctypes.c_void_p(torch.cuda.current_stream(dev).cuda_stream)
        self._bs = bs
        N, P32 = self.npatches, self.patch_size[0] // 32
        M = bs * N
        sh = self.sh
        new = lambda *s: torch.empty(s, dtype=torch.float32, device=dev)
        tok = new(M, 512)
        _lib.check(lib.omni_token_pack_f32(_p(d), _p(self.w["pos"]), _p(tok), M, N, P32 * P32, 32, self._s), "token_pack")
        normed = None
        pending = None
        for i in range(6):
            t = f"t{i}."
            if sh:
                if pending is not None:
                    tok, qkv = self._ln_gemm_parts(pending, t + "norm1.weight", t + "norm1.bias", 1e-5, t + "attn.qkv.w16", M, 1536)
                    pending = None
                elif normed is not None:
                    qkv = self._gemm_sh(normed, t + "attn.qkv.w16", None, M, 512, 1536)
                else:
                    qkv = self._ln_gemm_sh(tok, t + "norm1.weight", t + "norm1.bias", 1e-5, t + "attn.qkv.w16", None, M, 1536)
                att = new(M, 512)
                _lib.check(lib.omni_attention_qkv_sh(_p(qkv), _p(att), bs, N, self._s), "attention")
                tok = self._gemm_sh(att, t + "attn.proj.w16", t + "attn.proj.bias", M, 512, 512, res=tok)
                h = self._ln_gemm_sh(tok, t + "norm2.weight", t + "norm2.bias", 1e-5, t + "mlp.fc1.w16", t + "mlp.fc1.bias", M, 2048, act=ACT_GELU, out_sh=True)
                nxt = (f"t{i + 1}.norm1.weight", f"t{i + 1}.norm1.bias", 1e-5, True) if i < 5 else ("enc_norm.w", "enc_norm.b", 1e-6, False)
                tok, normed, pending = self._fc2_ln(h, t + "mlp.fc2.w16", t + "mlp.fc2.bias", M, tok, nxt)
                continue
            y = self._ln(tok, t + "norm1.weight", t + "norm1.bias", M, 1e-5)
            q = self._gemm(y, t + "attn.q.weight", None, M, 512, 512)
            kv = self._gemm(y, t + "attn.kv.weight", None, M, 512, 1024)
            att = new(M, 512)
            _lib.check(lib.omni_attention_f32(_p(q), _p(kv), _p(att), bs, N, self._s), "attention")
            tok = self._gemm(att, t + "attn.proj.weight", t + "attn.proj.bias", M, 512, 512, res=tok)
            y = self._ln(tok, t + "norm2.weight", t + "norm2.bias", M, 1e-5)
            h = self._gemm(y, t + "mlp.fc1.weight", t + "mlp.fc1.bias", M, 512, 2048, act=ACT_GELU)
            tok = self._gemm(h, t + "mlp.fc2.weight", t + "mlp.fc2.bias", M, 2048, 512, res=tok)
        if sh and pending is not None:
            parts, S, bkey, res_tok = pending
            tok_sum, tok = new(M, 512), new(M, 512)
            _lib.check(lib.omni_splitk_reduce_ln512(_p(parts), S, _p(self.w[bkey]), _p(res_tok), _p(tok_sum), _p(self.w["enc_norm.w"]), _p(self.w["enc_norm.b"]),
                                                    ctypes.c_float(1e-6), _p(tok), 0, M, self._s), "reduce+ln")
        else:
            tok = normed if (sh and normed is not None) else self._ln(tok, "enc_norm.w", "enc_norm.b", M, 1e-6)
        return tok

    def network(self, patches, point_feat, bs, confidence, out=None):
        lib = _lib.load()
        dev = patches.device
        self._s = ctypes.c_void_p(torch.cuda.current_stream(dev).cuda_stream)
        N, P = self.npatches, self.patch_size[0]
        M = bs * N
        self._bs = bs
        P2, P4, P8, P16, P32 = P // 2, P // 4, P // 8, P // 16, P // 32
        new = lambda *s: torch.empty(s, dtype=torch.float32, device=dev)
        conv1 = new(M, P2, P2, 64)
        sh = self.sh
        x = new(M, P4, P4, 64)
        pat = patches.view(M, 3, P, P)
        for m0, m1 in self._chunks(bs, N, self.front_chunk):
            Mc = m1 - m0
            if self.terms == 1 and P % 32:
                raise ValueError(f"precision f16x1 needs a patch size that is a multiple of 32 (got {P})")
            if sh and P % 32 == 0:
                _lib.check((lib.omni_stem_sh_f16x1 if self._x1 else lib.omni_stem_sh_f16x3)(_p(pat[m0:m1]), _p(self.w["stem.w16"]), _p(self.w["stem.b"]), _p(conv1[m0:m1]), Mc, P, self._s), "stem")
            else:
                _lib.check((lib.omni_stem_sh if sh else lib.omni_stem_f32)(_p(pat[m0:m1]), _p(self.w["stem.w"]), _p(self.w["stem.b"]),
                                                                            _p(conv1[m0:m1]), Mc, P, self._s), "stem")
            _lib.check((lib.omni_maxpool3x3s2_sh if sh else lib.omni_maxpool3x3s2_f32)(_p(conv1[m0:m1]), _p(x[m0:m1]), Mc, P2, P2, 64, self._s), "maxpool")
        feats = {}
        cin, size = 64, P4
        for lname, nblk, stride in _LAYERS:
            cout = {"layer1": 64, "layer2": 128, "layer3": 256, "layer4": 512}[lname]
            for i in range(nblk):
                p = f"{lname}.{i}"
                s = stride if i == 0 else 1
                ident = x
                if (p + ".ds.w") in self.w:
                    ident = self._conv(x, p + ".ds", M, size, size, cin, cout, 1, s, 0, ACT_NONE)
                y = self._conv(x, p + ".c1", M, size, size, cin, cout, 3, s, 1, ACT_RELU)
                size = (size + 2 - 3) // s + 1
                fold = sh and self.fold_point_feat and lname == "layer1" and i == nblk - 1
                x = self._conv(y, p + ".c2", M, size, size, cout, cout, 3, 1, 1, ACT_RELU, res=ident, post=point_feat if fold else None)
                cin = cout
            if lname == "layer1" and not (sh and self.fold_point_feat):
                _lib.check((lib.omni_add_period_sh if sh else lib.omni_add_period_f32)(
                    _p(x), _p(point_feat), ctypes.c_size_t(x.numel()), ctypes.c_size_t(point_feat.numel()), self._s), "add point_feat")
            feats[lname] = x
        layer1, layer2, layer3, layer4 = (feats[k] for k in ("layer1", "layer2", "layer3", "layer4"))
        if 32 * P32 * P32 != 512:
            raise RuntimeError(f"patch size {P}: token dim {32 * P32 * P32} != 512 — the reference network only exists at "
                               "patch size 128 (SURVEY.md finding 0.1)")
        d = self._conv(layer4, "down", M, P32, P32, 512, 32, 1, 1, 0, ACT_NONE, out_f32=True)
        tok = self.transformer(d, bs)
        _lib.check((lib.omni_add_hw_sh if sh else lib.omni_add_hw_f32)(_p(layer4), _p(tok), M, P32 * P32, 512, self._s), "token bias")
        x = self._up_conv_taps(layer4, "de_conv0_0", M, P32, P32, 512, 256, ACT_RELU)
        x = self._conv(x, "de_conv0_1", M, P16, P16, 256, 128, 3, 1, 1, ACT_RELU, x2=layer3, C2=256)
        x = self._up_conv_taps(x, "de_conv1_0", M, P16, P16, 128, 128, ACT_RELU)
        x = self._conv(x, "de_conv1_1", M, P8, P8, 128, 64, 3, 1, 1, ACT_RELU, x2=layer2, C2=128)
        x = self._up_conv(x, "de_conv2_0", M, P8, P8, 64, 64, ACT_RELU)
        x = self._conv(x, "de_conv2_1", M, P4, P4, 64, 64, 3, 1, 1, ACT_RELU, x2=layer1, C2=64)
        a, c = out if out is not None else (new(bs, N, 1, P, P), new(bs, N, 1, P, P) if confidence else None)
        av, cv = a.view(M, P, P), c.view(M, P, P) if c is not None else None
        fused = sh and self.fuse_heads and P % 32 == 0
        x_in, de4 = x, (None if fused else new(M, P, P, 32))
        for m0, m1 in self._chunks(bs, N, self.tail_chunk):
            Mc = m1 - m0
            x = self._up_conv(x_in[m0:m1], "de_conv3_0", Mc, P4, P4, 64, 64, ACT_RELU)
            x = self._conv(x, "de_conv3_1", Mc, P2, P2, 64, 32, 3, 1, 1, ACT_RELU, x2=conv1[m0:m1], C2=64)
            if fused:
                nb = int(lib.omni_up2_heads_scratch_bytes(Mc, P))
                hs = new((nb + 3) // 4)
                _lib.check((lib.omni_conv3x3_up2_heads_sh_f16x1 if self._x1 else lib.omni_conv3x3_up2_heads_sh_f16x3)(_p(x), _p(self.w["de_conv4_0.w16"]), _p(self.w["de_conv4_0.b"]), _p(self.w["heads.w16f"]),
                                                               ctypes.c_float(self.head_bias[0]), ctypes.c_float(self.head_bias[1]), _p(hs), ctypes.c_size_t(nb),
                                                               _p(av[m0:m1]), _p(cv[m0:m1]) if cv is not None else None, Mc, P, 1 if confidence else 0, self._s), "up+conv+heads")
                continue
            self._up_conv(x, "de_conv4_0", Mc, P2, P2, 32, 32, ACT_RELU, out_f32=True, out=de4[m0:m1])
            _lib.check(lib.omni_heads_f32(_p(de4[m0:m1]), _p(self.w["heads.w"]), ctypes.c_float(self.head_bias[0]), ctypes.c_float(self.head_bias[1]),
                                          _p(av[m0:m1]), _p(cv[m0:m1]) if cv is not None else None, Mc, P, 1 if confidence else 0, self._s), "heads")
        self.last = {"de_conv4_0": de4, "layer4": layer4}
        return a, c

    fuse_heads = os.environ.get("OMNI_FUSE_HEADS", "1") != "0"

    tail_chunk = 0
    front_chunk = 0

    @staticmethod
    def _chunks(bs, N, per):
        per = bs if per <= 0 else min(per, bs)
        return [(b0 * N, min(bs, b0 + per) * N) for b0 in range(0, bs, per)]

    def blend(self, a, c, erp_hw):
        P = self.patch_size
        if c is not None:
            return pers2equi_conf(a, c, self.fov, self.nrows, P, erp_hw, layout=_lib.LAYOUT_BNCHW)
        return pers2equi(a, self.fov, self.nrows, P, erp_hw, None, layout=_lib.LAYOUT_BNCHW)

    def mlp_points(self, name, xyz, depth, Mo):
        lib = _lib.load()
        P4 = self.patch_size[0] // 4
        out = torch.empty((Mo, P4, P4, 64), dtype=torch.float32, device=xyz.device)
        s = ctypes.c_void_p(torch.cuda.current_stream(xyz.device).cuda_stream)
        _lib.check(lib.omni_mlp_points_f32(_p(xyz), _p(depth), _p(self.w[name + ".w1"]), _p(self.w[name + ".b1"]),
                                           _p(self.w[name + ".w2"]), _p(self.w[name + ".b2"]), _p(out), Mo, self.npatches,
                                           P4 * P4, s), "mlp_points")
        return out

    def check_input(self, rgb):
        if not isinstance(rgb, torch.Tensor) or rgb.dim() != 4 or rgb.shape[1] != 3:
            raise ValueError("expected an RGB panorama batch [B,3,H,W]")
        if not rgb.is_cuda:
            raise ValueError("the model runs on an MI355X only (got a CPU tensor); there is no CPU path")
        if rgb.dtype != torch.float32:
            raise ValueError("float32 input expected")
        if _NPATCH[self.nrows] != self.npatches:
            raise ValueError("npatches does not match nrows")
```

Before: 4051 panoramas/s.

## Launch downsample 1x1 and first 3x3 conv of residual blocks as one paired kernel

Adds a paired conv entry point that runs a residual block's 3x3 c1 conv and its 1x1 downsample conv over the same input in a single launch. Each problem carries its own split-K plan and workspace slice, and the per-block setup is cached. This removes one launch per downsampling block and lets both convs share the input reads and fill the GPU together. It falls back to separate convs when unsupported or in batch-1 latency mode, and the large kernel-file rewrite risks changing the existing conv paths.

```diff
diff --git a/include/omnifusion.h b/include/omnifusion.h
--- a/include/omnifusion.h
+++ b/include/omnifusion.h
@@ -84,6 +84,13 @@
                             const void* res, void* dst, int fmt, int M, int H, int W, int C1, int C2, int Cout,
                             int KH, int KW, int stride, int pad, int act, int splitk, float* ws, size_t ws_bytes,
                             omni_stream_t stream);
+typedef struct omni_conv_sh_problem {
+    const void* wt16; const float* bias; const void* res; void* dst;
+    int fmt, Cout, KH, KW, stride, pad, act, splitk;
+    float* ws; size_t ws_bytes;
+} omni_conv_sh_problem_t;
+int omni_conv2d_sh_f16x3_pair_ws(const void* src, int M, int H, int W, int C,
+                                 const omni_conv_sh_problem_t* p0, const omni_conv_sh_problem_t* p1, omni_stream_t stream);
 int omni_gemm_rows_sh_f16x3(const void* x, const void* wt16r, const float* bias, const float* res, void* dst, int fmt,
                             int rows, int K, int N, int act, omni_stream_t stream);
 int omni_gemm_rows_pack(const void* wt16, void* wt16r, int N, int K, omni_stream_t stream);
diff --git a/omnifusion_amd/_lib.py b/omnifusion_amd/_lib.py
--- a/omnifusion_amd/_lib.py
+++ b/omnifusion_amd/_lib.py
@@ -12,6 +12,12 @@
 _lib = None
 
 
+class ConvShProblem(ctypes.Structure):
+    _fields_ = [("wt16", ctypes.c_void_p), ("bias", ctypes.c_void_p), ("res", ctypes.c_void_p), ("dst", ctypes.c_void_p),
+                ("fmt", ctypes.c_int), ("Cout", ctypes.c_int), ("KH", ctypes.c_int), ("KW", ctypes.c_int), ("stride", ctypes.c_int),
+                ("pad", ctypes.c_int), ("act", ctypes.c_int), ("splitk", ctypes.c_int), ("ws", ctypes.c_void_p), ("ws_bytes", ctypes.c_size_t)]
+
+
 class OmniLibraryMissing(ImportError):
     pass
 
@@ -24,7 +30,7 @@
     "omni_conv2d_nhwc_f32", "omni_stem_f32", "omni_maxpool3x3s2_f32", "omni_upsample_bilinear_f32",
     "omni_add_hw_f32", "omni_add_period_f32", "omni_token_pack_f32", "omni_layernorm512_f32",
     "omni_attention_f32", "omni_heads_f32", "omni_mlp_points_f32",
-    "omni_conv2d_nhwc_f16x3_ws", "omni_conv2d_sh_f16x3_ws", "omni_conv2d_sh_f16x3_post_ws", "omni_gemm_rows_sh_f16x3", "omni_gemm_rows_ln_sh_f16x3", "omni_gemm_rows_pack", "omni_conv3x3_up2_sh_f16x3", "omni_conv3x3_up2_heads_sh_f16x3", "omni_conv3x3_up2_heads_sh_f16x1", "omni_up2_heads_scratch_bytes", "omni_heads_pack_f16x3", "omni_sh_from_f32", "omni_sh_to_f32", "omni_sh_overflow",
+    "omni_conv2d_nhwc_f16x3_ws", "omni_conv2d_sh_f16x3_ws", "omni_conv2d_sh_f16x3_post_ws", "omni_conv2d_sh_f16x3_pair_ws", "omni_gemm_rows_sh_f16x3", "omni_gemm_rows_ln_sh_f16x3", "omni_gemm_rows_pack", "omni_conv3x3_up2_sh_f16x3", "omni_conv3x3_up2_heads_sh_f16x3", "omni_conv3x3_up2_heads_sh_f16x1", "omni_up2_heads_scratch_bytes", "omni_heads_pack_f16x3", "omni_sh_from_f32", "omni_sh_to_f32", "omni_sh_overflow",
     "omni_stem_sh", "omni_stem_sh_f16x3", "omni_stem_sh_f16x1", "omni_maxpool3x3s2_sh", "omni_upsample_bilinear_sh", "omni_up2_tapsum_sh", "omni_add_hw_sh", "omni_add_period_sh", "omni_layernorm512_sh", "omni_gemm_sh_f16x3_ln512_ws", "omni_gemm_rows_slices_sh_f16x3", "omni_gemm_rows_ln_parts_sh_f16x3", "omni_splitk_reduce_ln512", "omni_wino_input_sh", "omni_conv3x3_wino_sh_f16x3", "omni_attention_qkv_sh",
     "omni_conv2d_splitk_plan", "omni_conv2d_nhwc_f32_ws",
     "omni_masked_median_f32", "omni_depth_metrics_f32",
@@ -96,6 +102,7 @@
     lib.omni_geometry_terms_workspace_bytes.argtypes = [ci] * 3
     lib.omni_geometry_terms_f32.argtypes = [vp] * 4 + [ci] * 5 + [vp] * 3
     lib.omni_geometry_terms_grad_f32.argtypes = [vp] * 4 + [ci] * 4 + [vp] * 5
+    lib.omni_conv2d_sh_f16x3_pair_ws.argtypes = [vp] + [ci] * 4 + [ctypes.POINTER(ConvShProblem)] * 2 + [vp]
     for name in EXPORTS:
         getattr(lib, name)
     _lib = lib
diff --git a/omnifusion_amd/csrc/omni_conv_sh.hip b/omnifusion_amd/csrc/omni_conv_sh.hip
--- a/omnifusion_amd/csrc/omni_conv_sh.hip
+++ b/omnifusion_amd/csrc/omni_conv_sh.hip
@@ -10,436 +10,31 @@
 template <int BM, int BN, int WM, int WN, int NST = 3, int NL = 0, bool PP = false, bool WINO = false, bool X1 = false>
 __global__ __launch_bounds__(64 * (WM * WN + NL)) void conv_sh_kernel(ShConvArgs a)
 {
-    static_assert(!(WINO && X1), "Winograd: f16x3 only");
-    static_assert(!PP || (NL > 0 && WM * WN == 8 && NST >= 3), "ping-pong: eight matrix waves (two per SIMD) + loader waves, three stages");
-    static_assert(!WINO || (PP && BM / WM == 32 && BN / WN == 32), "Winograd: the ping-pong kernel with 32 x 32 wave tiles");
-    constexpr int NW = WM * WN, LW = NL > 0 ? NL : NW, RPP = 8 * LW;
-    constexpr int TM = BM / WM / 32, TN = BN / WN / 32;
-    constexpr int APASS = BM / RPP, BPASS = BN / RPP, LPS = APASS + BPASS;
-    static_assert(APASS >= 1 && BPASS >= 1, "a tile side must cover at least one DMA pass");
-    constexpr int A_BYTES = BM * 128, STAGE = (BM + BN) * 128;
-    __shared__ __attribute__((aligned(1024))) unsigned char lds[NST * STAGE];
-    __shared__ long long cst[OMNI_ABL(32768) ? 256 : 1];
-    const bool stamped = OMNI_ABL(32768) && blockIdx.x == 0 && blockIdx.y == 0 && a.ws != nullptr && a.splitk <= 1;
-    auto cstamp = [&](int k) { if (OMNI_ABL(32768) && stamped && (threadIdx.x & 63) == 0 && k < 256) cst[k] = clock64(); };
-    auto cdump = [&]() { if (OMNI_ABL(32768) && stamped && threadIdx.x == 0) for (int i = 0; i < 256; ++i) reinterpret_cast<long long*>(a.ws)[i] = cst[i]; };
-    if (threadIdx.x == 0) cstamp(0);
-
-    const int t = threadIdx.x, lane = t & 63;
-    const int wave = __builtin_amdgcn_readfirstlane(t >> 6);
-    const int wm = wave / WN, wn = wave % WN;
-    const bool loader = NL > 0 && wave >= NW;
-    const int iw = NL > 0 ? wave - NW : wave;
-    const int ntn = a.Cout / BN;
-    const int ntm = (a.rows + BM - 1) / BM;
-    const unsigned lb = a.noxcd ? blockIdx.x : omni_xcd_remap(blockIdx.x, gridDim.x);
-    const int tile_m = a.wt_major ? (int)(lb % (unsigned)ntm) : (int)(lb / (unsigned)ntn), tile_n = a.wt_major ? (int)(lb / (unsigned)ntm) : (int)(lb % (unsigned)ntn);
-    const int row0 = tile_m * BM, col0 = tile_n * BN;
-    const int G1 = a.C1 >> 5, G2 = a.C2 >> 5, G = G1 + G2;
-    const int ksteps = a.KH * a.KW * G;
-
-    const int gs = (lane & 15) ^ ((4 * iw + (lane >> 4)) & 15);
-    const int rl = 8 * iw + 2 * (lane >> 4) + (gs >> 3), pc16 = (gs & 7) * 16;
-    int pix[APASS];
-    unsigned vmask[APASS];
-#pragma unroll
-    for (int i = 0; i < APASS; ++i) {
-        const int r = row0 + rl + RPP * i;
-        vmask[i] = 0; pix[i] = 0;
-        if constexpr (WINO) {
-            if ((NL == 0 || loader) && r < a.rows) { pix[i] = r; vmask[i] = 0xffffu; }
-        } else
-        if ((NL == 0 || loader) && r < a.rows) {
-            const int hw = a.Ho * a.Wo;
-            const int m = r / hw, rem = r - m * hw;
-            const int oy = (rem / a.Wo) * a.stride - a.pad, ox = (rem % a.Wo) * a.stride - a.pad;
-            pix[i] = (m * a.H + oy) * a.W + ox;
-            unsigned vm = 0;
-#pragma unroll
-            for (int ky = 0; ky < 3; ++ky)
-#pragma unroll
-                for (int kx = 0; kx < 3; ++kx)
-                    if (ky < a.KH && kx < a.KW && (unsigned)(oy + ky) < (unsigned)a.H && (unsigned)(ox + kx) < (unsigned)a.W)
-                        vm |= 1u << (ky * a.KW + kx);
-            vmask[i] = vm;
-        }
-    }
-    const rsrc_t rs1 = make_rsrc(a.src1, (size_t)a.M * a.H * a.W * a.C1 * 4);
-    const rsrc_t rs2 = make_rsrc(a.src2 ? a.src2 : a.src1, a.src2 ? (size_t)a.M * a.H * a.W * a.C2 * 4 : 0);
-    const rsrc_t rsw = make_rsrc(a.wt, (size_t)a.Cout * ksteps * 128);
-    int wbase[BPASS];
-#pragma unroll
-    for (int i = 0; i < BPASS; ++i) wbase[i] = (col0 + rl + RPP * i) * ksteps * 128 + pc16;
-
-    int f_tap = 0, f_src = 0, f_gl = 0, f_ky = 0, f_kx = 0, f_gn = G1;
-    int voff[APASS];
-    auto refresh = [&]() {
-        const int cs4 = (f_src ? a.C2 : a.C1) * 4;
-        const int toff = (f_ky * a.W + f_kx) * cs4 + pc16;
-#pragma unroll
-        for (int i = 0; i < APASS; ++i)
-            voff[i] = ((vmask[i] >> f_tap) & 1u) ? pix[i] * cs4 + toff : (int)0x80000000;
-    };
-    auto seek = [&](int ks) {
-        f_tap = ks / G; const int g = ks - f_tap * G;
-        f_src = g >= G1; f_gl = f_src ? g - G1 : g; f_gn = f_src ? G2 : G1;
-        f_ky = f_tap / a.KW; f_kx = f_tap - f_ky * a.KW;
-        refresh();
-    };
-    auto issue_a = [&](auto slot_c) {
-        constexpr int SLOT = decltype(slot_c)::value;
-        unsigned char* sb = lds + SLOT * STAGE + iw * 1024;
-        const int so = f_gl * 128;
-        if (OMNI_ABL(128)) {}
-        else if (f_src) {
-#pragma unroll
-            for (int i = 0; i < APASS; ++i) dma16(rs2, sb + i * (1024 * LW), voff[i], so);
-        } else {
-#pragma unroll
-            for (int i = 0; i < APASS; ++i) dma16(rs1, sb + i * (1024 * LW), voff[i], so);
-        }
-    };
-    auto issue_b = [&](int ks, auto slot_c) {
-        constexpr int SLOT = decltype(slot_c)::value;
-        unsigned char* sb = lds + SLOT * STAGE + iw * 1024;
-        if (!OMNI_ABL(128)) {
-#pragma unroll
-            for (int i = 0; i < BPASS; ++i) dma16(rsw, sb + A_BYTES + i * (1024 * LW), wbase[i], ks * 128);
-        }
-        if (++f_gl == f_gn) {
-            f_gl = 0;
-            if (f_src == 0 && G2 > 0) { f_src = 1; f_gn = G2; }
-            else { f_src = 0; f_gn = G1; ++f_tap; if (++f_kx == a.KW) { f_kx = 0; ++f_ky; } }
-            refresh();
-        }
-    };
-    auto issue = [&](int ks, auto slot_c) { issue_a(slot_c); issue_b(ks, slot_c); };
-
-    f16v acc[TM][TN], acc1[TM][TN];
-#pragma unroll
-    for (int i = 0; i < TM; ++i)
-#pragma unroll
-        for (int j = 0; j < TN; ++j) { acc[i][j] = (f16v)(0.0f); acc1[i][j] = (f16v)(0.0f); }
-
-    int foa[4], fob[4];
-    {
-        const int r = lane & 31, v = r >> 1, h = lane >> 5;
-#pragma unroll
-        for (int k = 0; k < 4; ++k) {
-            const int f = v * 256 + ((((r & 1) * 8 + 2 * k + h) ^ v) * 16);
-            foa[k] = f + wm * (BM / WM) * 128;
-            fob[k] = f + A_BYTES + wn * (BN / WN) * 128;
-        }
-    }
-
-    int ks_begin = 0, ks_end = ksteps;
-    if (a.splitk > 1) {
-        const int per = (ksteps + a.splitk - 1) / a.splitk;
-        ks_begin = (int)blockIdx.y * per; ks_end = min(ksteps, ks_begin + per);
-    }
-    if (NL == 0 || loader) {
-        seek(ks_begin);
-        [&]<int... S>(std::integer_sequence<int, S...>) {
-            ((ks_begin + S < ks_end ? issue(ks_begin + S, std::integral_constant<int, S>()) : (void)0), ...);
-        }(std::make_integer_sequence<int, NST - 1>());
-    }
-    auto pbarrier = [&]() {
-        __builtin_amdgcn_sched_barrier(0);
-        __builtin_amdgcn_s_barrier();
-        asm volatile("" ::: "memory");
-        __builtin_amdgcn_sched_barrier(0);
-    };
-    if (loader) {
-        if constexpr (PP) {
-            auto lstep = [&](int ks, auto slot_c) {
-                constexpr int SLOT = decltype(slot_c)::value;
-                const int sk_ = 128 + 4 * (ks - ks_begin);
-                if (wave == NW && ks - ks_begin < 28) cstamp(sk_);
-                if (ks + NST - 2 < ks_end) wait_vm<(NST - 2) * LPS>();
-                else                       wait_vm<0>();
-                if (wave == NW && ks - ks_begin < 28) cstamp(sk_ + 1);
-                pbarrier();
-                if (wave == NW && ks - ks_begin < 28) cstamp(sk_ + 2);
-                if (ks + NST - 1 < ks_end) issue_a(std::integral_constant<int, (SLOT + NST - 1) % NST>());
-                if (wave == NW && ks - ks_begin < 28) cstamp(sk_ + 3);
-                pbarrier();
-                if (ks + NST - 1 < ks_end) issue_b(ks + NST - 1, std::integral_constant<int, (SLOT + NST - 1) % NST>());
-            };
-            int ks = ks_begin;
-            for (; ks + NST - 1 < ks_end; ks += NST) {
-                [&]<int... S>(std::integer_sequence<int, S...>) { (lstep(ks + S, std::integral_constant<int, S>()), ...); }
-                (std::make_integer_sequence<int, NST>());
-            }
-            [&]<int... S>(std::integer_sequence<int, S...>) {
-                ((ks + S < ks_end ? lstep(ks + S, std::integral_constant<int, S>()) : (void)0), ...);
-            }(std::make_integer_sequence<int, NST - 1>());
-            pbarrier();
-            if (!WINO && a.splitk <= 1 && a.dst_sh && !a.res_f32 && !a.post && a.epi_lds) __syncthreads();
-            return;
-        }
-        auto lstep = [&](int ks, auto slot_c) {
-            constexpr int SLOT = decltype(slot_c)::value;
-            const int sk_ = 128 + 4 * (ks - ks_begin);
-            if (wave == NW && ks - ks_begin < 28) cstamp(sk_);
-            if (ks + NST - 2 < ks_end) wait_vm<(NST - 2) * LPS>();
-            else                       wait_vm<0>();
-            if (wave == NW && ks - ks_begin < 28) cstamp(sk_ + 1);
-            __builtin_amdgcn_s_barrier();
-            asm volatile("" ::: "memory");
-            if (wave == NW && ks - ks_begin < 28) cstamp(sk_ + 2);
-            if (ks + NST - 1 < ks_end) issue(ks + NST - 1, std::integral_constant<int, (SLOT + NST - 1) % NST>());
-            if (wave == NW && ks - ks_begin < 28) cstamp(sk_ + 3);
-        };
-        int ks = ks_begin;
-        for (; ks + NST - 1 < ks_end; ks += NST) {
-            [&]<int... S>(std::integer_sequence<int, S...>) { (lstep(ks + S, std::integral_constant<int, S>()), ...); }
-            (std::make_integer_sequence<int, NST>());
-        }
-        [&]<int... S>(std::integer_sequence<int, S...>) {
-            ((ks + S < ks_end ? lstep(ks + S, std::integral_constant<int, S>()) : (void)0), ...);
-        }(std::make_integer_sequence<int, NST - 1>());
-        if (a.splitk <= 1 && a.dst_sh && !a.res_f32 && !a.post && a.epi_lds) __syncthreads();
-        return;
-    }
-
-    if constexpr (PP) {
-        const bool grp_b = wave >= NW / 2;
-        h8v ah[2][TM], al[2][TM], bh[2][TN], bl[2][TN];
-        auto reads = [&](auto slot_c) {
-            constexpr int SLOT = decltype(slot_c)::value;
-            const unsigned char* sl = lds + SLOT * STAGE;
-#pragma unroll
-            for (int kc = 0; kc < 2; ++kc) {
-#pragma unroll
-                for (int i = 0; i < TM; ++i) {
-                    ah[kc][i] = *reinterpret_cast<const h8v*>(sl + i * 4096 + foa[kc]);
-                    if constexpr (!X1) al[kc][i] = *reinterpret_cast<const h8v*>(sl + i * 4096 + foa[2 + kc]);
-                }
-#pragma unroll
-                for (int j = 0; j < TN; ++j) {
-                    bh[kc][j] = *reinterpret_cast<const h8v*>(sl + j * 4096 + fob[kc]);
-                    if constexpr (!X1) bl[kc][j] = *reinterpret_cast<const h8v*>(sl + j * 4096 + fob[2 + kc]);
-                }
-            }
-            wait_lds_reads();
-        };
-        auto mfmas = [&]() {
-            if constexpr (OMNI_PP_PRIO) __builtin_amdgcn_s_setprio(1);
-#pragma unroll
-            for (int kc = 0; kc < 2; ++kc)
-#pragma unroll
-                for (int i = 0; i < TM; ++i)
-#pragma unroll
-                    for (int j = 0; j < TN; ++j) {
-                        acc[i][j] = __builtin_amdgcn_mfma_f32_32x32x16_f16(bh[kc][j], ah[kc][i], acc[i][j], 0, 0, 0);
-                        if constexpr (!X1) {
-                            acc1[i][j] = __builtin_amdgcn_mfma_f32_32x32x16_f16(bl[kc][j], ah[kc][i], acc1[i][j], 0, 0, 0);
-                            acc1[i][j] = __builtin_amdgcn_mfma_f32_32x32x16_f16(bh[kc][j], al[kc][i], acc1[i][j], 0, 0, 0);
-                        }
-                    }
-            if constexpr (OMNI_PP_PRIO) __builtin_amdgcn_s_setprio(0);
-        };
-        f16v Y[WINO ? 4 : 1];
-        int wino_g = 0, wino_p = ks_begin / (G > 0 ? G : 1);
-        if constexpr (WINO) {
-#pragma unroll
-            for (int o = 0; o < 4; ++o) Y[o] = (f16v)(0.0f);
-        }
-        auto wino_fold = [&]() {
-            if constexpr (WINO) {
-                if (++wino_g < G) return;
-                wino_g = 0;
-                f16v m;
-#pragma unroll
-                for (int e = 0; e < 16; ++e) m[e] = fmaf(acc1[0][0][e], 4.8828125e-4f, acc[0][0][e]);
-#pragma unroll
-                for (int o = 0; o < 4; ++o) {
-                    const float c = wino_coef[wino_p][o];
-                    if (c != 0.0f) {
-#pragma unroll
-                        for (int e = 0; e < 16; ++e) Y[o][e] = fmaf(c, m[e], Y[o][e]);
-                    }
-                }
-                acc[0][0] = (f16v)(0.0f); acc1[0][0] = (f16v)(0.0f);
-                ++wino_p;
-            }
-        };
-        pbarrier();
-        if (!grp_b) {
-            auto stepa = [&](int ks, auto slot_c) {
-                if (wave == 0 && ks - ks_begin < 28) cstamp(8 + 4 * (ks - ks_begin));
-                reads(slot_c);
-                if (wave == 0 && ks - ks_begin < 28) cstamp(11 + 4 * (ks - ks_begin));
-                pbarrier();
-                if (wave == 0 && ks - ks_begin < 28) cstamp(9 + 4 * (ks - ks_begin));
-                mfmas();
-                wino_fold();
-                if (wave == 0 && ks - ks_begin < 28) cstamp(10 + 4 * (ks - ks_begin));
-                pbarrier();
-            };
-            int ks = ks_begin;
-            for (; ks + NST - 1 < ks_end; ks += NST) {
-                [&]<int... S>(std::integer_sequence<int, S...>) { (stepa(ks + S, std::integral_constant<int, S>()), ...); }
-                (std::make_integer_sequence<int, NST>());
-            }
-            [&]<int... S>(std::integer_sequence<int, S...>) {
-                ((ks + S < ks_end ? stepa(ks + S, std::integral_constant<int, S>()) : (void)0), ...);
-            }(std::make_integer_sequence<int, NST - 1>());
-        } else {
-            auto stepb = [&](int ks, auto slot_c) {
-                pbarrier();
-                reads(slot_c);
-                pbarrier();
-                mfmas();
-                wino_fold();
-            };
-            int ks = ks_begin;
-            for (; ks + NST - 1 < ks_end; ks += NST) {
-                [&]<int... S>(std::integer_sequence<int, S...>) { (stepb(ks + S, std::integral_constant<int, S>()), ...); }
-                (std::make_integer_sequence<int, NST>());
-            }
-            [&]<int... S>(std::integer_sequence<int, S...>) {
-                ((ks + S < ks_end ? stepb(ks + S, std::integral_constant<int, S>()) : (void)0), ...);
-            }(std::make_integer_sequence<int, NST - 1>());
-        }
-        if constexpr (WINO) {
-            const int tl = row0 + wm * (BM / WM) + (lane & 31);
-            if (tl >= a.rows) return;
-            const int per_img = a.wino_th * a.wino_tw, m = tl / per_img, rem = tl - m * per_img, ty = rem / a.wino_tw, tx = rem - ty * a.wino_tw;
-            const int cj[1] = {col0 + wn * (BN / WN)};
-#pragma unroll
-            for (int o = 0; o < 4; ++o) {
-                const size_t r = ((size_t)m * a.Ho + 2 * ty + (o >> 1)) * a.Wo + 2 * tx + (o & 1);
-                if (a.splitk > 1) {
-#pragma unroll
-                    for (int q = 0; q < 4; ++q) {
-                        f4v v; v.x = Y[o][4 * q]; v.y = Y[o][4 * q + 1]; v.z = Y[o][4 * q + 2]; v.w = Y[o][4 * q + 3];
-                        *reinterpret_cast<f4v*>(a.ws + ((size_t)blockIdx.y * a.wino_pix + r) * a.Cout + cj[0] + 8 * q + 4 * (lane >> 5)) = v;
-                    }
-                } else {
-                    const f16v ea[1] = {Y[o]}, eb[1] = {(f16v)(0.0f)};
-                    epilogue_row<1, 2>(ea, eb, a, r, cj, lane, a.dst_sh != 0);
-                }
-            }
-            return;
-        }
-    }
-    auto step = [&](int ks, auto slot_c) {
-        constexpr int SLOT = decltype(slot_c)::value;
-        if (NL == 0) {
-            if (ks + NST - 2 < ks_end) wait_vm<(NST - 2) * LPS>();
-            else                       wait_vm<0>();
-        }
-        if (wave == 0 && ks - ks_begin < 28) cstamp(8 + 4 * (ks - ks_begin));
-        wait_lds_reads();
-        if (!OMNI_ABL(256)) __builtin_amdgcn_s_barrier();
-        asm volatile("" ::: "memory");
-        if (wave == 0 && ks - ks_begin < 28) cstamp(9 + 4 * (ks - ks_begin));
-        const unsigned char* sl = lds + SLOT * STAGE;
-        h8v ah[2][TM], al[2][TM], bh[2][TN], bl[2][TN];
-        if (OMNI_ABL(512)) {
-#pragma unroll
-            for (int kc = 0; kc < 2; ++kc) {
-#pragma unroll
-                for (int i = 0; i < TM; ++i) { ah[kc][i] = (h8v)((_Float16)1.0f); al[kc][i] = ah[kc][i]; }
-#pragma unroll
-                for (int j = 0; j < TN; ++j) { bh[kc][j] = (h8v)((_Float16)1.0f); bl[kc][j] = bh[kc][j]; }
-            }
-        } else
-#pragma unroll
-        for (int kc = 0; kc < 2; ++kc) {
-#pragma unroll
-            for (int i = 0; i < TM; ++i) {
-                ah[kc][i] = *reinterpret_cast<const h8v*>(sl + i * 4096 + foa[kc]);
-                if constexpr (!X1) al[kc][i] = *reinterpret_cast<const h8v*>(sl + i * 4096 + foa[2 + kc]);
-            }
-#pragma unroll
-            for (int j = 0; j < TN; ++j) {
-                bh[kc][j] = *reinterpret_cast<const h8v*>(sl + j * 4096 + fob[kc]);
-                if constexpr (!X1) bl[kc][j] = *reinterpret_cast<const h8v*>(sl + j * 4096 + fob[2 + kc]);
-            }
-        }
-#pragma unroll
-        for (int kc = 0; kc < 2; ++kc) {
-            __builtin_amdgcn_sched_barrier(0);
-#pragma unroll
-            for (int i = 0; i < TM; ++i)
-#pragma unroll
-                for (int j = 0; j < TN; ++j) {
-                    if (!OMNI_ABL(64) && !OMNI_DBG(a, 64)) acc[i][j] = __builtin_amdgcn_mfma_f32_32x32x16_f16(bh[kc][j], ah[kc][i], acc[i][j], 0, 0, 0);
-                    else { acc[i][j][0] += (float)bh[kc][j][0] * (float)ah[kc][i][0]; }
-                    if constexpr (!X1) {
-                        if (!OMNI_ABL(16) && !OMNI_DBG(a, 16)) acc1[i][j] = __builtin_amdgcn_mfma_f32_32x32x16_f16(bl[kc][j], ah[kc][i], acc1[i][j], 0, 0, 0);
-                        if (!OMNI_ABL(32) && !OMNI_DBG(a, 32)) acc1[i][j] = __builtin_amdgcn_mfma_f32_32x32x16_f16(bh[kc][j], al[kc][i], acc1[i][j], 0, 0, 0);
-                    }
-                }
-            if (kc == 0) {
-                __builtin_amdgcn_sched_barrier(0);
-                if (NL == 0 && ks + NST - 1 < ks_end) issue(ks + NST - 1, std::integral_constant<int, (SLOT + NST - 1) % NST>());
-            }
-        }
-    };
-    if constexpr (!PP) {
-        int ks = ks_begin;
-        for (; ks + NST - 1 < ks_end; ks += NST) {
-            [&]<int... S>(std::integer_sequence<int, S...>) { (step(ks + S, std::integral_constant<int, S>()), ...); }
-            (std::make_integer_sequence<int, NST>());
-        }
-        [&]<int... S>(std::integer_sequence<int, S...>) {
-            ((ks + S < ks_end ? step(ks + S, std::integral_constant<int, S>()) : (void)0), ...);
-        }(std::make_integer_sequence<int, NST - 1>());
-    }
-
-    if (wave == 0) cstamp(1);
-    if (OMNI_ABL(4) || OMNI_DBG(a, 4)) return;
-    if (a.splitk <= 1 && a.dst_sh && !a.res_f32 && !a.post && a.epi_lds) {
-        static_assert(NW * 32 * (32 * TN + 4) * 4 <= NST * STAGE, "the transposition tiles must fit the K loop's buffers");
-        wait_lds_reads();
-        __syncthreads();
-        float* tile = reinterpret_cast<float*>(lds) + wave * (32 * (32 * TN + 4));
-        int c0[TN];
-#pragma unroll
-        for (int j = 0; j < TN; ++j) c0[j] = col0 + wn * (BN / WN) + j * 32;
-#pragma unroll
-        for (int i = 0; i < TM; ++i) {
-            const int r0 = row0 + wm * (BM / WM) + i * 32;
-            if (r0 < a.rows) epilogue_tile_lds<TN, false, X1>(acc[i], acc1[i], a, (size_t)r0, min(32, a.rows - r0), c0, lane, tile);
-            if (i + 1 < TM) asm volatile("s_waitcnt lgkmcnt(0)" ::: "memory");
-        }
-        if (OMNI_ABL(32768)) { if (wave == 0) cstamp(2); __syncthreads(); cdump(); }
-        return;
-    }
-#pragma unroll
-    for (int i = 0; i < TM; ++i) {
-        const int r = row0 + wm * (BM / WM) + i * 32 + (lane & 31);
-        if (r >= a.rows) continue;
-        if (a.splitk > 1) {
-#pragma unroll
-            for (int j = 0; j < TN; ++j)
-#pragma unroll
-                for (int q = 0; q < 4; ++q) {
-                    const int c = col0 + wn * (BN / WN) + j * 32 + 8 * q + 4 * (lane >> 5);
-                    f4v v;
-#pragma unroll
-                    for (int e = 0; e < 4; ++e) v[e] = acc_join<X1>(acc1[i][j][4 * q + e], acc[i][j][4 * q + e]);
-                    *reinterpret_cast<f4v*>(a.ws + ((size_t)blockIdx.y * a.rows + r) * a.Cout + c) = v;
-                }
-        } else {
-            if constexpr (NL > 0 && TN > 1) {
-#pragma unroll
-                for (int j = 0; j < TN; ++j) {
-                    const f16v ea[1] = {acc[i][j]}, eb[1] = {acc1[i][j]};
-                    const int cj[1] = {col0 + wn * (BN / WN) + j * 32};
-                    epilogue_row<1, 2, X1>(ea, eb, a, (size_t)r, cj, lane, a.dst_sh != 0);
-                }
-            } else {
-                int c0[TN];
-#pragma unroll
-                for (int j = 0; j < TN; ++j) c0[j] = col0 + wn * (BN / WN) + j * 32;
-                epilogue_row<TN, 4, X1>(acc[i], acc1[i], a, (size_t)r, c0, lane, a.dst_sh != 0);
-            }
-        }
-    }
+#define OMNI_CONV_BX blockIdx.x
+#define OMNI_CONV_NBX gridDim.x
+#define OMNI_CONV_BY blockIdx.y
+#include "omni_conv_sh_body.h"
+#undef OMNI_CONV_BX
+#undef OMNI_CONV_NBX
+#undef OMNI_CONV_BY
+}
+
+struct ShConvPairArgs { ShConvArgs p[2]; unsigned nb0; unsigned tiles[2]; };
+template <int BM, int BN, int WM, int WN, int NST, int NL, bool PP, bool X1>
+__global__ __launch_bounds__(64 * (WM * WN + NL)) void conv_sh_pair_kernel(ShConvPairArgs pa)
+{
+    const unsigned second = blockIdx.x >= pa.nb0 ? 1u : 0u;
+    const unsigned local = blockIdx.x - (second ? pa.nb0 : 0u), tiles = pa.tiles[second];
+    const unsigned slab = local / tiles, tile = local - slab * tiles;
+    const ShConvArgs& a = pa.p[second];
+    constexpr bool WINO = false;
+#define OMNI_CONV_BX tile
+#define OMNI_CONV_NBX tiles
+#define OMNI_CONV_BY slab
+#include "omni_conv_sh_body.h"
+#undef OMNI_CONV_BX
+#undef OMNI_CONV_NBX
+#undef OMNI_CONV_BY
 }
 
 __global__ __launch_bounds__(256) void sh_splitk_reduce_kernel(const float* __restrict__ ws, const float* __restrict__ bias,
@@ -520,6 +115,10 @@
                           const void* res, void* dst, int fmt, int M, int H, int W, int C1, int C2, int Cout,
                           int KH, int KW, int stride, int pad, int act, int splitk, float* ws, size_t ws_bytes,
                           const float* post, size_t post_elems, omni_stream_t stream, bool reduce = true);
+static int conv_sh_fill(ShConvArgs& a, const void* src1, const void* src2, const void* wt16, const float* bias,
+                        const void* res, void* dst, int fmt, int M, int H, int W, int C1, int C2, int Cout,
+                        int KH, int KW, int stride, int pad, int act, int splitk, float* ws, size_t ws_bytes,
+                        const float* post, size_t post_elems);
 extern "C" int omni_conv2d_sh_f16x3_ws(const void* src1, const void* src2, const void* wt16, const float* bias,
                                        const void* res, void* dst, int fmt, int M, int H, int W, int C1, int C2, int Cout,
                                        int KH, int KW, int stride, int pad, int act, int splitk, float* ws, size_t ws_bytes,
@@ -610,13 +209,34 @@
                           int KH, int KW, int stride, int pad, int act, int splitk, float* ws, size_t ws_bytes,
                           const float* post, size_t post_elems, omni_stream_t stream, bool reduce)
 {
+    ShConvArgs a;
+    const int rc = conv_sh_fill(a, src1, src2, wt16, bias, res, dst, fmt, M, H, W, C1, C2, Cout, KH, KW, stride, pad, act, splitk, ws, ws_bytes, post, post_elems);
+    if (rc != OMNI_OK) return rc;
+    const long long rows = a.rows;
+    hipStream_t s = (hipStream_t)stream;
+    if (fmt & 8) conv_sh_select<true>(a, fmt, s);
+    else         conv_sh_select<false>(a, fmt, s);
+    OMNI_HIP(hipGetLastError());
+    if (a.splitk > 1 && reduce) {
+        const size_t n4 = (size_t)rows * Cout / 4;
+        hipLaunchKernelGGL(sh_splitk_reduce_kernel, dim3((unsigned)((n4 + 255) / 256)), dim3(256), 0, s, (const float*)ws, bias, res, dst,
+                           n4, Cout, a.splitk, (size_t)rows * Cout, act, a.dst_sh, a.res_f32);
+        OMNI_HIP(hipGetLastError());
+    }
+    return OMNI_OK;
+}
+
+static int conv_sh_fill(ShConvArgs& a, const void* src1, const void* src2, const void* wt16, const float* bias,
+                        const void* res, void* dst, int fmt, int M, int H, int W, int C1, int C2, int Cout,
+                        int KH, int KW, int stride, int pad, int act, int splitk, float* ws, size_t ws_bytes,
+                        const float* post, size_t post_elems)
+{
     const int dst_sh = fmt & 1;
     if (!src1 || !wt16 || !dst) OMNI_FAIL(OMNI_ERR_INVALID, "omni_conv2d_sh: null pointer");
     if (C1 <= 0 || C1 % 32 || C2 < 0 || C2 % 32 || Cout <= 0 || Cout % 32 || (C2 > 0 && !src2))
         OMNI_FAIL(OMNI_ERR_INVALID, "omni_conv2d_sh: channels must be multiples of 32");
     if (M <= 0 || H <= 0 || W <= 0 || KH <= 0 || KW <= 0 || KH > 3 || KW > 3 || stride <= 0 || pad < 0)
         OMNI_FAIL(OMNI_ERR_INVALID, "omni_conv2d_sh: bad shape (kernels up to 3x3)");
-    ShConvArgs a;
     a.src1 = src1; a.src2 = src2; a.wt = wt16; a.bias = bias; a.res = res; a.dst = dst; a.dst_sh = dst_sh; a.res_f32 = (fmt >> 1) & 1;
     a.dbg = 0; a.noxcd = omni_options().conv_noxcd; a.wt_major = 0; a.epi_lds = omni_options().conv_epi_lds && !(fmt & 4);
 #ifdef OMNI_DEBUG_BUILD
@@ -646,14 +266,58 @@
         if (a.splitk > 1) OMNI_FAIL(OMNI_ERR_UNSUPPORTED, "omni_conv2d_sh: no post-activation addend with split-K");
         a.post_rows = (unsigned)(post_elems / (size_t)Cout);
     }
+    return OMNI_OK;
+}
+
+extern "C" int omni_conv2d_sh_f16x3_pair_ws(const void* src, int M, int H, int W, int C,
+                                            const omni_conv_sh_problem_t* p0, const omni_conv_sh_problem_t* p1, omni_stream_t stream)
+{
+    if (!p0 || !p1) OMNI_FAIL(OMNI_ERR_INVALID, "omni_conv2d_sh_pair: null problem");
+    const omni_conv_sh_problem_t* pr[2] = {p0, p1};
+    ShConvPairArgs pa;
+    for (int i = 0; i < 2; ++i) {
+        const omni_conv_sh_problem_t& q = *pr[i];
+        const int rc = conv_sh_fill(pa.p[i], src, nullptr, q.wt16, q.bias, q.res, q.dst, q.fmt, M, H, W, C, 0, q.Cout, q.KH, q.KW, q.stride, q.pad, q.act,
+                                    q.splitk, q.ws, q.ws_bytes, nullptr, 0);
+        if (rc != OMNI_OK) return rc;
+    }
+    const ShConvArgs &a0 = pa.p[0], &a1 = pa.p[1];
+    if (a0.rows != a1.rows) OMNI_FAIL(OMNI_ERR_UNSUPPORTED, "omni_conv2d_sh_pair: the two problems must have the same number of output rows");
+    if ((p0->fmt ^ p1->fmt) & 8) OMNI_FAIL(OMNI_ERR_UNSUPPORTED, "omni_conv2d_sh_pair: the two problems must run the same arithmetic mode (fmt bit 3)");
+    if (a0.splitk > 1 && a1.splitk > 1) {
+        const char *b0 = (const char*)a0.ws, *b1 = (const char*)a1.ws;
+        const size_t n0 = (size_t)a0.splitk * a0.rows * a0.Cout * 4, n1 = (size_t)a1.splitk * a1.rows * a1.Cout * 4;
+        if (b0 < b1 + n1 && b1 < b0 + n0) OMNI_FAIL(OMNI_ERR_INVALID, "omni_conv2d_sh_pair: the two split-K workspaces overlap");
+    }
+    const int tile = omni_options().conv_sh_tile;
+    const bool halo0 = a0.splitk <= 1 && a0.KH == 3 && a0.KW == 3 && a0.stride == 1 && a0.pad == 1 && !omni_options().conv_nohalo &&
+                       ((W % HT_W == 0 && H % 4 == 0) || (H == W && (W == 16 || W == 8)));
+    if (halo0 || (tile >= 0 && tile != 8) || a0.Cout % 128 || a1.Cout % 128)
+        OMNI_FAIL(OMNI_ERR_UNSUPPORTED, "omni_conv2d_sh_pair: no paired form of the kernel this shape and these options select");
+    const bool x1 = (p0->fmt & 8) != 0;
+    const long long r256 = (a0.rows + 255) / 256, r128 = (a0.rows + 127) / 128;
+    const bool big = r256 * (a0.Cout / 128) * a0.splitk >= std::max(1, omni_options().conv_big_blocks);
+    const int BM = big ? 256 : 128;
+    for (int i = 0; i < 2; ++i) pa.tiles[i] = (unsigned)((big ? r256 : r128) * (pa.p[i].Cout / 128));
+    pa.nb0 = pa.tiles[0] * (unsigned)a0.splitk;
+    const unsigned grid = pa.nb0 + pa.tiles[1] * (unsigned)a1.splitk;
     hipStream_t s = (hipStream_t)stream;
-    if (fmt & 8) conv_sh_select<true>(a, fmt, s);
-    else         conv_sh_select<false>(a, fmt, s);
-    OMNI_HIP(hipGetLastError());
-    if (a.splitk > 1 && reduce) {
-        const size_t n4 = (size_t)rows * Cout / 4;
-        hipLaunchKernelGGL(sh_splitk_reduce_kernel, dim3((unsigned)((n4 + 255) / 256)), dim3(256), 0, s, (const float*)ws, bias, res, dst,
-                           n4, Cout, a.splitk, (size_t)rows * Cout, act, a.dst_sh, a.res_f32);
+    const bool pp = omni_options().conv_pingpong != 0;
+#define OMNI_PAIR(X1_) \
+    do { \
+        if (BM == 256) hipLaunchKernelGGL((conv_sh_pair_kernel<256, 128, 4, 2, 3, 0, false, X1_>), dim3(grid), dim3(64 * 8), 0, s, pa); \
+        else if (pp)   hipLaunchKernelGGL((conv_sh_pair_kernel<128, 128, 4, 2, 3, 4, true, X1_>), dim3(grid), dim3(64 * 12), 0, s, pa); \
+        else           hipLaunchKernelGGL((conv_sh_pair_kernel<128, 128, 4, 2, 3, 4, false, X1_>), dim3(grid), dim3(64 * 12), 0, s, pa); \
+    } while (0)
+    if (x1) OMNI_PAIR(true); else OMNI_PAIR(false);
+#undef OMNI_PAIR
+    OMNI_HIP(hipGetLastError());
+    for (int i = 0; i < 2; ++i) {
+        const ShConvArgs& a = pa.p[i];
+        if (a.splitk <= 1) continue;
+        const size_t n4 = (size_t)a.rows * a.Cout / 4;
+        hipLaunchKernelGGL(sh_splitk_reduce_kernel, dim3((unsigned)((n4 + 255) / 256)), dim3(256), 0, s, (const float*)a.ws, a.bias, a.res, a.dst,
+                           n4, a.Cout, a.splitk, (size_t)a.rows * a.Cout, a.act, a.dst_sh, a.res_f32);
         OMNI_HIP(hipGetLastError());
     }
     return OMNI_OK;
diff --git a/omnifusion_amd/csrc/omni_conv_sh_body.h b/omnifusion_amd/csrc/omni_conv_sh_body.h
--- /dev/null
+++ b/omnifusion_amd/csrc/omni_conv_sh_body.h
@@ -0,0 +1,430 @@
+    static_assert(!(WINO && X1), "Winograd: f16x3 only");
+    static_assert(!PP || (NL > 0 && WM * WN == 8 && NST >= 3), "ping-pong: eight matrix waves (two per SIMD) + loader waves, three stages");
+    static_assert(!WINO || (PP && BM / WM == 32 && BN / WN == 32), "Winograd: the ping-pong kernel with 32 x 32 wave tiles");
+    constexpr int NW = WM * WN, LW = NL > 0 ? NL : NW, RPP = 8 * LW;
+    constexpr int TM = BM / WM / 32, TN = BN / WN / 32;
+    constexpr int APASS = BM / RPP, BPASS = BN / RPP, LPS = APASS + BPASS;
+    static_assert(APASS >= 1 && BPASS >= 1, "a tile side must cover at least one DMA pass");
+    constexpr int A_BYTES = BM * 128, STAGE = (BM + BN) * 128;
+    __shared__ __attribute__((aligned(1024))) unsigned char lds[NST * STAGE];
+    __shared__ long long cst[OMNI_ABL(32768) ? 256 : 1];
+    const bool stamped = OMNI_ABL(32768) && OMNI_CONV_BX == 0 && OMNI_CONV_BY == 0 && a.ws != nullptr && a.splitk <= 1;
+    auto cstamp = [&](int k) { if (OMNI_ABL(32768) && stamped && (threadIdx.x & 63) == 0 && k < 256) cst[k] = clock64(); };
+    auto cdump = [&]() { if (OMNI_ABL(32768) && stamped && threadIdx.x == 0) for (int i = 0; i < 256; ++i) reinterpret_cast<long long*>(a.ws)[i] = cst[i]; };
+    if (threadIdx.x == 0) cstamp(0);
+
+    const int t = threadIdx.x, lane = t & 63;
+    const int wave = __builtin_amdgcn_readfirstlane(t >> 6);
+    const int wm = wave / WN, wn = wave % WN;
+    const bool loader = NL > 0 && wave >= NW;
+    const int iw = NL > 0 ? wave - NW : wave;
+    const int ntn = a.Cout / BN;
+    const int ntm = (a.rows + BM - 1) / BM;
+    const unsigned lb = a.noxcd ? OMNI_CONV_BX : omni_xcd_remap(OMNI_CONV_BX, OMNI_CONV_NBX);
+    const int tile_m = a.wt_major ? (int)(lb % (unsigned)ntm) : (int)(lb / (unsigned)ntn), tile_n = a.wt_major ? (int)(lb / (unsigned)ntm) : (int)(lb % (unsigned)ntn);
+    const int row0 = tile_m * BM, col0 = tile_n * BN;
+    const int G1 = a.C1 >> 5, G2 = a.C2 >> 5, G = G1 + G2;
+    const int ksteps = a.KH * a.KW * G;
+
+    const int gs = (lane & 15) ^ ((4 * iw + (lane >> 4)) & 15);
+    const int rl = 8 * iw + 2 * (lane >> 4) + (gs >> 3), pc16 = (gs & 7) * 16;
+    int pix[APASS];
+    unsigned vmask[APASS];
+#pragma unroll
+    for (int i = 0; i < APASS; ++i) {
+        const int r = row0 + rl + RPP * i;
+        vmask[i] = 0; pix[i] = 0;
+        if constexpr (WINO) {
+            if ((NL == 0 || loader) && r < a.rows) { pix[i] = r; vmask[i] = 0xffffu; }
+        } else
+        if ((NL == 0 || loader) && r < a.rows) {
+            const int hw = a.Ho * a.Wo;
+            const int m = r / hw, rem = r - m * hw;
+            const int oy = (rem / a.Wo) * a.stride - a.pad, ox = (rem % a.Wo) * a.stride - a.pad;
+            pix[i] = (m * a.H + oy) * a.W + ox;
+            unsigned vm = 0;
+#pragma unroll
+            for (int ky = 0; ky < 3; ++ky)
+#pragma unroll
+                for (int kx = 0; kx < 3; ++kx)
+                    if (ky < a.KH && kx < a.KW && (unsigned)(oy + ky) < (unsigned)a.H && (unsigned)(ox + kx) < (unsigned)a.W)
+                        vm |= 1u << (ky * a.KW + kx);
+            vmask[i] = vm;
+        }
+    }
+    const rsrc_t rs1 = make_rsrc(a.src1, (size_t)a.M * a.H * a.W * a.C1 * 4);
+    const rsrc_t rs2 = make_rsrc(a.src2 ? a.src2 : a.src1, a.src2 ? (size_t)a.M * a.H * a.W * a.C2 * 4 : 0);
+    const rsrc_t rsw = make_rsrc(a.wt, (size_t)a.Cout * ksteps * 128);
+    int wbase[BPASS];
+#pragma unroll
+    for (int i = 0; i < BPASS; ++i) wbase[i] = (col0 + rl + RPP * i) * ksteps * 128 + pc16;
+
+    int f_tap = 0, f_src = 0, f_gl = 0, f_ky = 0, f_kx = 0, f_gn = G1;
+    int voff[APASS];
+    auto refresh = [&]() {
+        const int cs4 = (f_src ? a.C2 : a.C1) * 4;
+        const int toff = (f_ky * a.W + f_kx) * cs4 + pc16;
+#pragma unroll
+        for (int i = 0; i < APASS; ++i)
+            voff[i] = ((vmask[i] >> f_tap) & 1u) ? pix[i] * cs4 + toff : (int)0x80000000;
+    };
+    auto seek = [&](int ks) {
+        f_tap = ks / G; const int g = ks - f_tap * G;
+        f_src = g >= G1; f_gl = f_src ? g - G1 : g; f_gn = f_src ? G2 : G1;
+        f_ky = f_tap / a.KW; f_kx = f_tap - f_ky * a.KW;
+        refresh();
+    };
+    auto issue_a = [&](auto slot_c) {
+        constexpr int SLOT = decltype(slot_c)::value;
+        unsigned char* sb = lds + SLOT * STAGE + iw * 1024;
+        const int so = f_gl * 128;
+        if (OMNI_ABL(128)) {}
+        else if (f_src) {
+#pragma unroll
+            for (int i = 0; i < APASS; ++i) dma16(rs2, sb + i * (1024 * LW), voff[i], so);
+        } else {
+#pragma unroll
+            for (int i = 0; i < APASS; ++i) dma16(rs1, sb + i * (1024 * LW), voff[i], so);
+        }
+    };
+    auto issue_b = [&](int ks, auto slot_c) {
+        constexpr int SLOT = decltype(slot_c)::value;
+        unsigned char* sb = lds + SLOT * STAGE + iw * 1024;
+        if (!OMNI_ABL(128)) {
+#pragma unroll
+            for (int i = 0; i < BPASS; ++i) dma16(rsw, sb + A_BYTES + i * (1024 * LW), wbase[i], ks * 128);
+        }
+        if (++f_gl == f_gn) {
+            f_gl = 0;
+            if (f_src == 0 && G2 > 0) { f_src = 1; f_gn = G2; }
+            else { f_src = 0; f_gn = G1; ++f_tap; if (++f_kx == a.KW) { f_kx = 0; ++f_ky; } }
+            refresh();
+        }
+    };
+    auto issue = [&](int ks, auto slot_c) { issue_a(slot_c); issue_b(ks, slot_c); };
+
+    f16v acc[TM][TN], acc1[TM][TN];
+#pragma unroll
+    for (int i = 0; i < TM; ++i)
+#pragma unroll
+        for (int j = 0; j < TN; ++j) { acc[i][j] = (f16v)(0.0f); acc1[i][j] = (f16v)(0.0f); }
+
+    int foa[4], fob[4];
+    {
+        const int r = lane & 31, v = r >> 1, h = lane >> 5;
+#pragma unroll
+        for (int k = 0; k < 4; ++k) {
+            const int f = v * 256 + ((((r & 1) * 8 + 2 * k + h) ^ v) * 16);
+            foa[k] = f + wm * (BM / WM) * 128;
+            fob[k] = f + A_BYTES + wn * (BN / WN) * 128;
+        }
+    }
+
+    int ks_begin = 0, ks_end = ksteps;
+    if (a.splitk > 1) {
+        const int per = (ksteps + a.splitk - 1) / a.splitk;
+        ks_begin = (int)OMNI_CONV_BY * per; ks_end = min(ksteps, ks_begin + per);
+    }
+    if (NL == 0 || loader) {
+        seek(ks_begin);
+        [&]<int... S>(std::integer_sequence<int, S...>) {
+            ((ks_begin + S < ks_end ? issue(ks_begin + S, std::integral_constant<int, S>()) : (void)0), ...);
+        }(std::make_integer_sequence<int, NST - 1>());
+    }
+    auto pbarrier = [&]() {
+        __builtin_amdgcn_sched_barrier(0);
+        __builtin_amdgcn_s_barrier();
+        asm volatile("" ::: "memory");
+        __builtin_amdgcn_sched_barrier(0);
+    };
+    if (loader) {
+        if constexpr (PP) {
+            auto lstep = [&](int ks, auto slot_c) {
+                constexpr int SLOT = decltype(slot_c)::value;
+                const int sk_ = 128 + 4 * (ks - ks_begin);
+                if (wave == NW && ks - ks_begin < 28) cstamp(sk_);
+                if (ks + NST - 2 < ks_end) wait_vm<(NST - 2) * LPS>();
+                else                       wait_vm<0>();
+                if (wave == NW && ks - ks_begin < 28) cstamp(sk_ + 1);
+                pbarrier();
+                if (wave == NW && ks - ks_begin < 28) cstamp(sk_ + 2);
+                if (ks + NST - 1 < ks_end) issue_a(std::integral_constant<int, (SLOT + NST - 1) % NST>());
+                if (wave == NW && ks - ks_begin < 28) cstamp(sk_ + 3);
+                pbarrier();
+                if (ks + NST - 1 < ks_end) issue_b(ks + NST - 1, std::integral_constant<int, (SLOT + NST - 1) % NST>());
+            };
+            int ks = ks_begin;
+            for (; ks + NST - 1 < ks_end; ks += NST) {
+                [&]<int... S>(std::integer_sequence<int, S...>) { (lstep(ks + S, std::integral_constant<int, S>()), ...); }
+                (std::make_integer_sequence<int, NST>());
+            }
+            [&]<int... S>(std::integer_sequence<int, S...>) {
+                ((ks + S < ks_end ? lstep(ks + S, std::integral_constant<int, S>()) : (void)0), ...);
+            }(std::make_integer_sequence<int, NST - 1>());
+            pbarrier();
+            if (!WINO && a.splitk <= 1 && a.dst_sh && !a.res_f32 && !a.post && a.epi_lds) __syncthreads();
+            return;
+        }
+        auto lstep = [&](int ks, auto slot_c) {
+            constexpr int SLOT = decltype(slot_c)::value;
+            const int sk_ = 128 + 4 * (ks - ks_begin);
+            if (wave == NW && ks - ks_begin < 28) cstamp(sk_);
+            if (ks + NST - 2 < ks_end) wait_vm<(NST - 2) * LPS>();
+            else                       wait_vm<0>();
+            if (wave == NW && ks - ks_begin < 28) cstamp(sk_ + 1);
+            __builtin_amdgcn_s_barrier();
+            asm volatile("" ::: "memory");
+            if (wave == NW && ks - ks_begin < 28) cstamp(sk_ + 2);
+            if (ks + NST - 1 < ks_end) issue(ks + NST - 1, std::integral_constant<int, (SLOT + NST - 1) % NST>());
+            if (wave == NW && ks - ks_begin < 28) cstamp(sk_ + 3);
+        };
+        int ks = ks_begin;
+        for (; ks + NST - 1 < ks_end; ks += NST) {
+            [&]<int... S>(std::integer_sequence<int, S...>) { (lstep(ks + S, std::integral_constant<int, S>()), ...); }
+            (std::make_integer_sequence<int, NST>());
+        }
+        [&]<int... S>(std::integer_sequence<int, S...>) {
+            ((ks + S < ks_end ? lstep(ks + S, std::integral_constant<int, S>()) : (void)0), ...);
+        }(std::make_integer_sequence<int, NST - 1>());
+        if (a.splitk <= 1 && a.dst_sh && !a.res_f32 && !a.post && a.epi_lds) __syncthreads();
+        return;
+    }
+
+    if constexpr (PP) {
+        const bool grp_b = wave >= NW / 2;
+        h8v ah[2][TM], al[2][TM], bh[2][TN], bl[2][TN];
+        auto reads = [&](auto slot_c) {
+            constexpr int SLOT = decltype(slot_c)::value;
+            const unsigned char* sl = lds + SLOT * STAGE;
+#pragma unroll
+            for (int kc = 0; kc < 2; ++kc) {
+#pragma unroll
+                for (int i = 0; i < TM; ++i) {
+                    ah[kc][i] = *reinterpret_cast<const h8v*>(sl + i * 4096 + foa[kc]);
+                    if constexpr (!X1) al[kc][i] = *reinterpret_cast<const h8v*>(sl + i * 4096 + foa[2 + kc]);
+                }
+#pragma unroll
+                for (int j = 0; j < TN; ++j) {
+                    bh[kc][j] = *reinterpret_cast<const h8v*>(sl + j * 4096 + fob[kc]);
+                    if constexpr (!X1) bl[kc][j] = *reinterpret_cast<const h8v*>(sl + j * 4096 + fob[2 + kc]);
+                }
+            }
+            wait_lds_reads();
+        };
+        auto mfmas = [&]() {
+            if constexpr (OMNI_PP_PRIO) __builtin_amdgcn_s_setprio(1);
+#pragma unroll
+            for (int kc = 0; kc < 2; ++kc)
+#pragma unroll
+                for (int i = 0; i < TM; ++i)
+#pragma unroll
+                    for (int j = 0; j < TN; ++j) {
+                        acc[i][j] = __builtin_amdgcn_mfma_f32_32x32x16_f16(bh[kc][j], ah[kc][i], acc[i][j], 0, 0, 0);
+                        if constexpr (!X1) {
+                            acc1[i][j] = __builtin_amdgcn_mfma_f32_32x32x16_f16(bl[kc][j], ah[kc][i], acc1[i][j], 0, 0, 0);
+                            acc1[i][j] = __builtin_amdgcn_mfma_f32_32x32x16_f16(bh[kc][j], al[kc][i], acc1[i][j], 0, 0, 0);
+                        }
+                    }
+            if constexpr (OMNI_PP_PRIO) __builtin_amdgcn_s_setprio(0);
+        };
+        f16v Y[WINO ? 4 : 1];
+        int wino_g = 0, wino_p = ks_begin / (G > 0 ? G : 1);
+        if constexpr (WINO) {
+#pragma unroll
+            for (int o = 0; o < 4; ++o) Y[o] = (f16v)(0.0f);
+        }
+        auto wino_fold = [&]() {
+            if constexpr (WINO) {
+                if (++wino_g < G) return;
+                wino_g = 0;
+                f16v m;
+#pragma unroll
+                for (int e = 0; e < 16; ++e) m[e] = fmaf(acc1[0][0][e], 4.8828125e-4f, acc[0][0][e]);
+#pragma unroll
+                for (int o = 0; o < 4; ++o) {
+                    const float c = wino_coef[wino_p][o];
+                    if (c != 0.0f) {
+#pragma unroll
+                        for (int e = 0; e < 16; ++e) Y[o][e] = fmaf(c, m[e], Y[o][e]);
+                    }
+                }
+                acc[0][0] = (f16v)(0.0f); acc1[0][0] = (f16v)(0.0f);
+                ++wino_p;
+            }
+        };
+        pbarrier();
+        if (!grp_b) {
+            auto stepa = [&](int ks, auto slot_c) {
+                if (wave == 0 && ks - ks_begin < 28) cstamp(8 + 4 * (ks - ks_begin));
+                reads(slot_c);
+                if (wave == 0 && ks - ks_begin < 28) cstamp(11 + 4 * (ks - ks_begin));
+                pbarrier();
+                if (wave == 0 && ks - ks_begin < 28) cstamp(9 + 4 * (ks - ks_begin));
+                mfmas();
+                wino_fold();
+                if (wave == 0 && ks - ks_begin < 28) cstamp(10 + 4 * (ks - ks_begin));
+                pbarrier();
+            };
+            int ks = ks_begin;
+            for (; ks + NST - 1 < ks_end; ks += NST) {
+                [&]<int... S>(std::integer_sequence<int, S...>) { (stepa(ks + S, std::integral_constant<int, S>()), ...); }
+                (std::make_integer_sequence<int, NST>());
+            }
+            [&]<int... S>(std::integer_sequence<int, S...>) {
+                ((ks + S < ks_end ? stepa(ks + S, std::integral_constant<int, S>()) : (void)0), ...);
+            }(std::make_integer_sequence<int, NST - 1>());
+        } else {
+            auto stepb = [&](int ks, auto slot_c) {
+                pbarrier();
+                reads(slot_c);
+                pbarrier();
+                mfmas();
+                wino_fold();
+            };
+            int ks = ks_begin;
+            for (; ks + NST - 1 < ks_end; ks += NST) {
+                [&]<int... S>(std::integer_sequence<int, S...>) { (stepb(ks + S, std::integral_constant<int, S>()), ...); }
+                (std::make_integer_sequence<int, NST>());
+            }
+            [&]<int... S>(std::integer_sequence<int, S...>) {
+                ((ks + S < ks_end ? stepb(ks + S, std::integral_constant<int, S>()) : (void)0), ...);
+            }(std::make_integer_sequence<int, NST - 1>());
+        }
+        if constexpr (WINO) {
+            const int tl = row0 + wm * (BM / WM) + (lane & 31);
+            if (tl >= a.rows) return;
+            const int per_img = a.wino_th * a.wino_tw, m = tl / per_img, rem = tl - m * per_img, ty = rem / a.wino_tw, tx = rem - ty * a.wino_tw;
+            const int cj[1] = {col0 + wn * (BN / WN)};
+#pragma unroll
+            for (int o = 0; o < 4; ++o) {
+                const size_t r = ((size_t)m * a.Ho + 2 * ty + (o >> 1)) * a.Wo + 2 * tx + (o & 1);
+                if (a.splitk > 1) {
+#pragma unroll
+                    for (int q = 0; q < 4; ++q) {
+                        f4v v; v.x = Y[o][4 * q]; v.y = Y[o][4 * q + 1]; v.z = Y[o][4 * q + 2]; v.w = Y[o][4 * q + 3];
+                        *reinterpret_cast<f4v*>(a.ws + ((size_t)OMNI_CONV_BY * a.wino_pix + r) * a.Cout + cj[0] + 8 * q + 4 * (lane >> 5)) = v;
+                    }
+                } else {
+                    const f16v ea[1] = {Y[o]}, eb[1] = {(f16v)(0.0f)};
+                    epilogue_row<1, 2>(ea, eb, a, r, cj, lane, a.dst_sh != 0);
+                }
+            }
+            return;
+        }
+    }
+    auto step = [&](int ks, auto slot_c) {
+        constexpr int SLOT = decltype(slot_c)::value;
+        if (NL == 0) {
+            if (ks + NST - 2 < ks_end) wait_vm<(NST - 2) * LPS>();
+            else                       wait_vm<0>();
+        }
+        if (wave == 0 && ks - ks_begin < 28) cstamp(8 + 4 * (ks - ks_begin));
+        wait_lds_reads();
+        if (!OMNI_ABL(256)) __builtin_amdgcn_s_barrier();
+        asm volatile("" ::: "memory");
+        if (wave == 0 && ks - ks_begin < 28) cstamp(9 + 4 * (ks - ks_begin));
+        const unsigned char* sl = lds + SLOT * STAGE;
+        h8v ah[2][TM], al[2][TM], bh[2][TN], bl[2][TN];
+        if (OMNI_ABL(512)) {
+#pragma unroll
+            for (int kc = 0; kc < 2; ++kc) {
+#pragma unroll
+                for (int i = 0; i < TM; ++i) { ah[kc][i] = (h8v)((_Float16)1.0f); al[kc][i] = ah[kc][i]; }
+#pragma unroll
+                for (int j = 0; j < TN; ++j) { bh[kc][j] = (h8v)((_Float16)1.0f); bl[kc][j] = bh[kc][j]; }
+            }
+        } else
+#pragma unroll
+        for (int kc = 0; kc < 2; ++kc) {
+#pragma unroll
+            for (int i = 0; i < TM; ++i) {
+                ah[kc][i] = *reinterpret_cast<const h8v*>(sl + i * 4096 + foa[kc]);
+                if constexpr (!X1) al[kc][i] = *reinterpret_cast<const h8v*>(sl + i * 4096 + foa[2 + kc]);
+            }
+#pragma unroll
+            for (int j = 0; j < TN; ++j) {
+                bh[kc][j] = *reinterpret_cast<const h8v*>(sl + j * 4096 + fob[kc]);
+                if constexpr (!X1) bl[kc][j] = *reinterpret_cast<const h8v*>(sl + j * 4096 + fob[2 + kc]);
+            }
+        }
+#pragma unroll
+        for (int kc = 0; kc < 2; ++kc) {
+            __builtin_amdgcn_sched_barrier(0);
+#pragma unroll
+            for (int i = 0; i < TM; ++i)
+#pragma unroll
+                for (int j = 0; j < TN; ++j) {
+                    if (!OMNI_ABL(64) && !OMNI_DBG(a, 64)) acc[i][j] = __builtin_amdgcn_mfma_f32_32x32x16_f16(bh[kc][j], ah[kc][i], acc[i][j], 0, 0, 0);
+                    else { acc[i][j][0] += (float)bh[kc][j][0] * (float)ah[kc][i][0]; }
+                    if constexpr (!X1) {
+                        if (!OMNI_ABL(16) && !OMNI_DBG(a, 16)) acc1[i][j] = __builtin_amdgcn_mfma_f32_32x32x16_f16(bl[kc][j], ah[kc][i], acc1[i][j], 0, 0, 0);
+                        if (!OMNI_ABL(32) && !OMNI_DBG(a, 32)) acc1[i][j] = __builtin_amdgcn_mfma_f32_32x32x16_f16(bh[kc][j], al[kc][i], acc1[i][j], 0, 0, 0);
+                    }
+                }
+            if (kc == 0) {
+                __builtin_amdgcn_sched_barrier(0);
+                if (NL == 0 && ks + NST - 1 < ks_end) issue(ks + NST - 1, std::integral_constant<int, (SLOT + NST - 1) % NST>());
+            }
+        }
+    };
+    if constexpr (!PP) {
+        int ks = ks_begin;
+        for (; ks + NST - 1 < ks_end; ks += NST) {
+            [&]<int... S>(std::integer_sequence<int, S...>) { (step(ks + S, std::integral_constant<int, S>()), ...); }
+            (std::make_integer_sequence<int, NST>());
+        }
+        [&]<int... S>(std::integer_sequence<int, S...>) {
+            ((ks + S < ks_end ? step(ks + S, std::integral_constant<int, S>()) : (void)0), ...);
+        }(std::make_integer_sequence<int, NST - 1>());
+    }
+
+    if (wave == 0) cstamp(1);
+    if (OMNI_ABL(4) || OMNI_DBG(a, 4)) return;
+    if (a.splitk <= 1 && a.dst_sh && !a.res_f32 && !a.post && a.epi_lds) {
+        static_assert(NW * 32 * (32 * TN + 4) * 4 <= NST * STAGE, "the transposition tiles must fit the K loop's buffers");
+        wait_lds_reads();
+        __syncthreads();
+        float* tile = reinterpret_cast<float*>(lds) + wave * (32 * (32 * TN + 4));
+        int c0[TN];
+#pragma unroll
+        for (int j = 0; j < TN; ++j) c0[j] = col0 + wn * (BN / WN) + j * 32;
+#pragma unroll
+        for (int i = 0; i < TM; ++i) {
+            const int r0 = row0 + wm * (BM / WM) + i * 32;
+            if (r0 < a.rows) epilogue_tile_lds<TN, false, X1>(acc[i], acc1[i], a, (size_t)r0, min(32, a.rows - r0), c0, lane, tile);
+            if (i + 1 < TM) asm volatile("s_waitcnt lgkmcnt(0)" ::: "memory");
+        }
+        if (OMNI_ABL(32768)) { if (wave == 0) cstamp(2); __syncthreads(); cdump(); }
+        return;
+    }
+#pragma unroll
+    for (int i = 0; i < TM; ++i) {
+        const int r = row0 + wm * (BM / WM) + i * 32 + (lane & 31);
+        if (r >= a.rows) continue;
+        if (a.splitk > 1) {
+#pragma unroll
+            for (int j = 0; j < TN; ++j)
+#pragma unroll
+                for (int q = 0; q < 4; ++q) {
+                    const int c = col0 + wn * (BN / WN) + j * 32 + 8 * q + 4 * (lane >> 5);
+                    f4v v;
+#pragma unroll
+                    for (int e = 0; e < 4; ++e) v[e] = acc_join<X1>(acc1[i][j][4 * q + e], acc[i][j][4 * q + e]);
+                    *reinterpret_cast<f4v*>(a.ws + ((size_t)OMNI_CONV_BY * a.rows + r) * a.Cout + c) = v;
+                }
+        } else {
+            if constexpr (NL > 0 && TN > 1) {
+#pragma unroll
+                for (int j = 0; j < TN; ++j) {
+                    const f16v ea[1] = {acc[i][j]}, eb[1] = {acc1[i][j]};
+                    const int cj[1] = {col0 + wn * (BN / WN) + j * 32};
+                    epilogue_row<1, 2, X1>(ea, eb, a, (size_t)r, cj, lane, a.dst_sh != 0);
+                }
+            } else {
+                int c0[TN];
+#pragma unroll
+                for (int j = 0; j < TN; ++j) c0[j] = col0 + wn * (BN / WN) + j * 32;
+                epilogue_row<TN, 4, X1>(acc[i], acc1[i], a, (size_t)r, c0, lane, a.dst_sh != 0);
+            }
+        }
+    }
diff --git a/omnifusion_amd/model/_engine.py b/omnifusion_amd/model/_engine.py
--- a/omnifusion_amd/model/_engine.py
+++ b/omnifusion_amd/model/_engine.py
@@ -303,6 +303,40 @@
 
     fold_point_feat = True
     fuse_up = True
+
+    pair_ds = True
+
+    def _conv_pair(self, x, p, M, size, cin, cout, stride):
+        if self._bs == 1 and self.latency_plan:
+            return None, None
+        lib = _lib.load()
+        cache = self.__dict__.setdefault("_pairs", {})
+        ck = (p, M, self._bs, size, self._x1)
+        c = cache.get(ck)
+        if c is None or c[5] is not self.w:
+            So = (size + 2 - 3) // stride + 1
+            if (size - 1) // stride + 1 != So:
+                return None, None
+            rows = M * So * So
+            plan = lambda ksteps: max(1, int(lib.omni_conv2d_splitk_plan(ctypes.c_longlong(rows // self._bs * self.NOMINAL_BATCH), cout, ksteps)))
+            S1, Sd = plan(9 * cin // 32), plan(cin // 32)
+            n1 = (S1 * rows * cout * 4 + 255) // 256 * 256 if S1 > 1 else 0
+            nd = Sd * rows * cout * 4 if Sd > 1 else 0
+            prob = lambda key, k, pad, act, S, nb: _lib.ConvShProblem(
+                self.w[key + ".w16"].data_ptr(), self.w[key + ".b"].data_ptr(), None, None, 1 | self._x1, cout, k, k, stride, pad, act, S, None, nb)
+            c = cache[ck] = (prob(p + ".c1", 3, 1, ACT_RELU, S1, n1), prob(p + ".ds", 1, 0, ACT_NONE, Sd, nd), n1, nd, So, self.w)
+        p0, p1, n1, nd, So, _ = c
+        y = torch.empty((M, So, So, cout), dtype=torch.float32, device=x.device)
+        ident = torch.empty((M, So, So, cout), dtype=torch.float32, device=x.device)
+        p0.dst, p1.dst = y.data_ptr(), ident.data_ptr()
+        if n1 + nd:
+            base = self._workspace(n1 + nd, x.device)[0].data_ptr()
+            p0.ws, p1.ws = (base if n1 else None), (base + n1 if nd else None)
+        rc = lib.omni_conv2d_sh_f16x3_pair_ws(_p(x), M, size, size, cin, ctypes.byref(p0), ctypes.byref(p1), self._s)
+        if rc == _lib.OMNI_ERR_UNSUPPORTED:
+            return None, None
+        _lib.check(rc, "conv2d " + p + ".c1+ds")
+        return y, ident
 
     def _up_conv(self, x, key, M, H, Wd, C, Cout, act, out_f32=False, out=None):
         Ho, Wo = 2 * H, 2 * Wd
@@ -403,10 +437,14 @@
             for i in range(nblk):
                 p = f"{lname}.{i}"
                 s = stride if i == 0 else 1
-                ident = x
+                ident, y = x, None
                 if (p + ".ds.w") in self.w:
-                    ident = self._conv(x, p + ".ds", M, size, size, cin, cout, 1, s, 0, ACT_NONE)
-                y = self._conv(x, p + ".c1", M, size, size, cin, cout, 3, s, 1, ACT_RELU)
+                    if sh and self.pair_ds:
+                        y, ident = self._conv_pair(x, p, M, size, cin, cout, s)
+                    if y is None:
+                        ident = self._conv(x, p + ".ds", M, size, size, cin, cout, 1, s, 0, ACT_NONE)
+                if y is None:
+                    y = self._conv(x, p + ".c1", M, size, size, cin, cout, 3, s, 1, ACT_RELU)
                 size = (size + 2 - 3) // s + 1
                 fold = sh and self.fold_point_feat and lname == "layer1" and i == nblk - 1
                 x = self._conv(y, p + ".c2", M, size, size, cout, cout, 3, 1, 1, ACT_RELU, res=ident, post=point_feat if fold else None)
```

Measured after the change: 4075 panoramas/s, median of 6. Within noise of the previous version (+0.6%).
